# jglaser/metadynamics-plugin

Measured on AMD Instinct MI355X. Metric: particle_cv_evals_per_s, higher is better.
Workload: dtype f32; 1 GPU; 1xMI355X: 10^6 particles, 2 lamellar CVs (8 Fourier modes each), 256^2 bias grid, well-tempered; particles_per_gpu=1000000, particles_global=1000000, n_cv=2, modes_per_cv=8, grid=256x256, stride=1, fast_trig=1, fast_trig_library_default=1, driver=host, mode=single

## Files before the change

metadynamics-plugin_amd/csrc/fused.hip:

```cpp
#include <hip/hip_runtime.h>
#include <hip/hip_ext.h>

#ifdef MTD_STAMPS
__device__ unsigned long long g_stamps[64];
#define MTD_STAMP(slot, cond)                                                   \
    do                                                                          \
        {                                                                       \
        if (cond) g_stamps[slot] = wall_clock64();                              \
        } while (0)
extern "C" int mtd_debug_read_stamps(unsigned long long *host)
    {
    return (int)hipMemcpyFromSymbol(host, HIP_SYMBOL(g_stamps), sizeof(unsigned long long) * 64);
    }
#else
#define MTD_STAMP(slot, cond) do { } while (0)
#endif

#include "lamellar_host.hpp"
#include "metad_host.hpp"
#include "comm_host.hpp"

#include <cstdlib>
#include <cstring>
#include <map>
#include <mutex>
#include <utility>
#include <vector>

namespace
{

using namespace mtd;

constexpr int FCV_THREADS = 512;
constexpr int FCV_UNROLL = 4;
constexpr int FF_THREADS = 256;
constexpr int FF_UNROLL = 2;

template<typename S4, int NCV, bool FAST, bool COMM, bool ORTHO, int U = FCV_UNROLL>
__global__ __launch_bounds__(FCV_THREADS) void k_fused_cv(const LamKArgs a, const S4 *__restrict__ postype, const unsigned int N,
                                                          double *partials, const MetadCfg c,
                                                          const unsigned int n_apply_blocks, const CommK ck)
    {
    __shared__ float s_coeff[MTD_MAX_CV * MTD_MAX_TYPES];
    __shared__ double s_wave[(FCV_THREADS / MTD_WAVE) * NCV];
    __shared__ double s_red[16];
    __shared__ ModeTables s_mt;

    MTD_STAMP(0, blockIdx.x == 0 && threadIdx.x == 0);
    MTD_STAMP(3, blockIdx.x == n_apply_blocks && threadIdx.x == 0);
    if (blockIdx.x < n_apply_blocks)
        {
        const unsigned int b0 = blockIdx.x * FCV_THREADS;
        apply_cells(c, b0, min(c.len, b0 + FCV_THREADS), blockIdx.x == 0, s_red);
        MTD_STAMP(1, blockIdx.x == 0 && threadIdx.x == 0);
        return;
        }
    const unsigned int block_id = blockIdx.x - n_apply_blocks;
    const unsigned int n_blocks = gridDim.x - n_apply_blocks;

    RawGroup<S4, U> first;
    const S4 *src = N ? postype : (const S4 *)partials;
    lam_load_group_nc<S4, U>(src, N ? N : 1u, block_id * FCV_THREADS + threadIdx.x, n_blocks * FCV_THREADS, first);
    const CvTableRegs tab = stage_cv_tables_request(a);
    stage_cv_tables_store(tab, s_coeff, s_mt);
    __syncthreads();
    MTD_STAMP(4, block_id == 0 && threadIdx.x == 0);
    float acc[NCV];
#pragma unroll
    for (int i = 0; i < NCV; ++i) acc[i] = 0.0f;
    lam_cv_accumulate<S4, NCV, FAST, U, ORTHO>(a, postype, N, block_id * FCV_THREADS + threadIdx.x, n_blocks * FCV_THREADS,
                                               s_coeff, s_mt, first, acc);
    MTD_STAMP(5, block_id == 0 && threadIdx.x == 0);
    lam_cv_block_reduce<NCV>(acc, s_wave, partials, block_id);
    MTD_STAMP(6, block_id == 0 && threadIdx.x == 0);
    if (COMM)
        {
        constexpr int NS = NCV < 3 ? NCV : 3;
        if (threadIdx.x < NS)
            ll_store(ck.ll + ((size_t)block_id * NS + threadIdx.x) * 2, ck.seq, partials[block_id * NCV + threadIdx.x]);
        if (block_id != 0 || threadIdx.x >= MTD_WAVE) return;
        double v[3] = { 0.0, 0.0, 0.0 };
        const bool expired = ll_collect_wave<NS>(ck, n_blocks, v);
        MTD_STAMP(7, threadIdx.x == 0);
        double tot[3] = { 0.0, 0.0, 0.0 };
#pragma unroll
        for (int i = 0; i < NS; ++i)
            {
            const double t = wave_sum(v[i]);
            tot[i] = expired ? comm_poison() : t;
            }
        MTD_STAMP(8, threadIdx.x == 0);
        comm_send_wave(ck, tot, NS);
        MTD_STAMP(9, threadIdx.x == 0);
        }
    }

constexpr int FF_STREAM_WAVES = FF_THREADS / MTD_WAVE - 1;
constexpr int FF_STREAM_THREADS = FF_STREAM_WAVES * MTD_WAVE;
constexpr int FF_U = 4;
template<typename S4, int NCV, bool FAST> struct ff_groups { static constexpr int value = 1; };
template<> struct ff_groups<float4, 1, true> { static constexpr int value = 2; };
template<> struct ff_groups<float4, 2, true> { static constexpr int value = 2; };
template<> struct ff_groups<float4, 1, false> { static constexpr int value = 2; };
template<> struct ff_groups<double4, 1, true> { static constexpr int value = 2; };
template<> struct ff_groups<double4, 1, false> { static constexpr int value = 2; };

template<typename S4, int NCV, bool FAST, int GROUPS, bool COMM, bool ORTHO>
__global__ __launch_bounds__(FF_THREADS, 4) void k_fused_force(const LamKArgs a, const S4 *__restrict__ postype, const ForcePtrs out,
                                                            const unsigned int N, const double two_over_n, const MetadCfg c,
                                                            const int deposit, const unsigned int n_grid_blocks, const CommK ck)
    {
    __shared__ ChainResult s_chain;
    __shared__ float s_wcoef[MTD_MAX_CV * MTD_MAX_TYPES];
    __shared__ double s_red[16];
    __shared__ ModeTables s_mt;

    const int wave = threadIdx.x >> 6;
    const int lane = threadIdx.x & 63;
    const bool grid_block = blockIdx.x < n_grid_blocks;
    const unsigned int block_id = blockIdx.x - n_grid_blocks;
    const unsigned int n_blocks = gridDim.x - n_grid_blocks;
    const unsigned int stride = n_blocks * FF_STREAM_THREADS;
    const unsigned int first = block_id * FF_STREAM_THREADS + (wave - 1) * MTD_WAVE + lane;
    const unsigned int first1 = first + FF_U * stride;

    ForceRegs<NCV, FF_U> R, R1;
    MTD_STAMP(16, blockIdx.x == 0 && threadIdx.x == 0);
    MTD_STAMP(24, blockIdx.x == n_grid_blocks && threadIdx.x == 0);
    constexpr int NCH = CHAIN_MAX_CV;
    ChainPre<NCH> pre;
    constexpr bool early = !COMM;
    float4 th = make_float4(0.f, 0.f, 0.f, 0.f), tq = th;
    float tc = 0.0f;
    if (wave == 0)
        {
        if (!grid_block)
            {
            if (lane < (int)a.n_modes)
                {
                th = a.h[lane];
                tq = a.q[lane];
                }
            if (lane < NCV * MTD_MAX_TYPES) tc = a.coeff[lane / MTD_MAX_TYPES][lane % MTD_MAX_TYPES];
            }
        if (early)
            chain_preload<NCH>(c, pre);
        else
            chain_preload<NCH, false>(c, pre);
        }
    RawGroup<S4, FF_U> raw0;
    if (wave != 0 && !grid_block && N) lam_force_request<S4, FF_U>(postype, N, first, stride, raw0);
    if (!grid_block)
        {
        if (wave == 0)
            {
            if (lane < (int)a.n_modes)
                {
                s_mt.h[lane] = th;
                s_mt.q[lane] = tq;
                }
            if (lane < NCV * MTD_MAX_TYPES) s_wcoef[lane] = tc;
            }
        lds_barrier();
        }
    MTD_STAMP(25, blockIdx.x == n_grid_blocks && threadIdx.x == 0);
    if (wave == 0)
        {
        ChainResult r;
        if constexpr (early)
            {
            double vi[3];
#pragma unroll
            for (int i = 0; i < NCH; ++i) vi[i] = (pre.x[i][0] + pre.x[i][1]) + (pre.x[i][2] + pre.x[i][3]);
            r = chain_wave(c, deposit != 0, true, nullptr, nullptr, false, &pre.patch, pre.patch_ok != 0, true, vi[0], vi[1], vi[2]);
            }
        else
            r = chain_wave(c, deposit != 0, true, &ck, nullptr, false, &pre.patch, pre.patch_ok != 0);
        MTD_STAMP(17, blockIdx.x == 0 && threadIdx.x == 0);
        MTD_STAMP(26, blockIdx.x == n_grid_blocks && threadIdx.x == 0);
        if (lane == 0) chain_share(s_chain, r);
        if (!grid_block && lane < NCV * MTD_MAX_TYPES)
            {
            const unsigned int cv = lane / MTD_MAX_TYPES;
            const unsigned int gs = cv < a.n_cv ? a.slot[cv] : 0u;
            const double b = gs == 0 ? r.bias[0] : (gs == 1 ? r.bias[1] : r.bias[2]);
            s_wcoef[lane] = (cv < a.n_cv) ? (float)((double)s_wcoef[lane] * b * two_over_n) : 0.0f;
            }
        }
    else if (!grid_block && N)
        {
        RawGroup<S4, FF_U> raw1;
        if (GROUPS > 1) lam_force_request<S4, FF_U>(postype, N, first1, stride, raw1);
        lam_force_unscaled_from<S4, NCV, FAST, FF_U, ORTHO>(a, N, first, stride, s_mt, raw0, R);
        if (GROUPS > 1) lam_force_unscaled_from<S4, NCV, FAST, FF_U, ORTHO>(a, N, first1, stride, s_mt, raw1, R1);
        MTD_STAMP(27, blockIdx.x == n_grid_blocks && threadIdx.x == 64);
        }
    lds_barrier();
    MTD_STAMP(18, blockIdx.x == 0 && threadIdx.x == 0);
    MTD_STAMP(28, blockIdx.x == n_grid_blocks && threadIdx.x == 64);

    if (grid_block)
        {
        const double2 sums = grid_first_pass_cells_256(c, s_chain, blockIdx.x);
        MTD_STAMP(19, blockIdx.x == 0 && threadIdx.x == 0);
        grid_first_pass_sums_256(c, blockIdx.x, sums, s_red);
        MTD_STAMP(20, blockIdx.x == 0 && threadIdx.x == 0);
        }
    else if (wave != 0 && N)
        {
        lam_force_store<S4, NCV, FF_U>(a, out, first, stride, s_wcoef, R);
        if (GROUPS > 1) lam_force_store<S4, NCV, FF_U>(a, out, first1, stride, s_wcoef, R1);
        MTD_STAMP(29, blockIdx.x == n_grid_blocks && threadIdx.x == 64);
        }

    if (blockIdx.x == 0 && wave == 0) publish_step(c, s_chain, deposit, nullptr, COMM ? &ck : nullptr);
    }

template<typename S4, bool FAST>
__global__ __launch_bounds__(FF_THREADS) void k_fused_force_general(const LamKArgs a, const S4 *__restrict__ postype, const ForcePtrs out,
                                                            const unsigned int N, const double two_over_n, const MetadCfg c,
                                                            const int deposit, const unsigned int n_grid_blocks)
    {
    __shared__ EvalShared sh;
    __shared__ float s_wcoef[MTD_MAX_CV * MTD_MAX_TYPES];
    __shared__ double s_red[16];
    __shared__ ModeTables s_mt;

    load_modes(a, s_mt, true);
    reduce_cv_sources(c, sh.cv, s_red);
    __syncthreads();
    evaluate_bias(c, sh, deposit != 0, true);

    if (blockIdx.x < n_grid_blocks)
        {
        const unsigned int g = blockIdx.x * FF_THREADS + threadIdx.x;
        double s1 = 0.0, s2 = 0.0;
        if (g < c.len)
            {
            const double dV = (c.W * sh.scal) * exp(-gauss_exponent(c, g, sh.cv));
            c.grid_delta[g] = dV;
            unsigned int hd = c.hist_delta[g];
            if (sh.on_grid && g == sh.bin)
                {
                hd += 1;
                c.hist_delta[g] = hd;
                c.sigma_grid_delta[g] += c.det_sigma;
                c.hist_gauss_delta[g] += 1;
                }
            const double R = c.rew[g] + (double)hd;
            c.rew[g] = R;
            s1 = R * dV;
            s2 = R;
            }
        s1 = block_sum(s1, s_red);
        s2 = block_sum(s2, s_red);
        if (threadIdx.x == 0)
            {
            c.gpart[2 * blockIdx.x] = s1;
            c.gpart[2 * blockIdx.x + 1] = s2;
            }
        }

    if (blockIdx.x == 0)
        {
        if (threadIdx.x < c.n_cv)
            {
            c.st->cv[threadIdx.x] = sh.cv[threadIdx.x];
            c.st->bias[threadIdx.x] = sh.bias[threadIdx.x];
            }
        if (threadIdx.x == 0)
            {
            c.st->V = sh.res[0];
            c.st->bin = sh.bin;
            c.st->on_grid = (unsigned int)sh.on_grid;
            if (deposit)
                c.st->scal = sh.scal;
            else
                {
                c.st->w = sh.res[1];
                if (sh.on_grid) c.hist_delta[sh.bin] += 1;
                }
            if (sh.oob[0]) c.st->n_oob += (deposit && c.mode == MTD_MODE_WELL_TEMPERED) ? 2 : 1;
            }
        }
    if (blockIdx.x < n_grid_blocks) return;

    const unsigned int block_id = blockIdx.x - n_grid_blocks;
    const unsigned int n_blocks = gridDim.x - n_grid_blocks;
    for (unsigned int i = threadIdx.x; i < MTD_MAX_CV * MTD_MAX_TYPES; i += blockDim.x)
        {
        const unsigned int cv = i / MTD_MAX_TYPES;
        const double b = cv < a.n_cv ? sh.bias[a.slot[cv]] : 0.0;
        s_wcoef[i] = (float)((double)a.coeff[cv][i % MTD_MAX_TYPES] * b * two_over_n);
        }
    __syncthreads();
    lam_force_pass<S4, FAST, FF_UNROLL>(a, postype, out, N, block_id * FF_THREADS + threadIdx.x, n_blocks * FF_THREADS, s_wcoef, s_mt);
    }

struct ForceProfile
    {
    std::vector<hipEvent_t> ev;
    size_t used = 0;
    };
ForceProfile g_force_profile;
std::mutex g_force_profile_mutex;

bool force_profile_next(hipEvent_t &start, hipEvent_t &stop)
    {
    std::lock_guard<std::mutex> lock(g_force_profile_mutex);
    ForceProfile &p = g_force_profile;
    if (p.used + 2 > p.ev.size()) return false;
    start = p.ev[p.used];
    stop = p.ev[p.used + 1];
    p.used += 2;
    return true;
    }

template<typename F> int with_fused_cv_kernel(int dtype, bool fast, bool ortho, bool comm, unsigned int n_cv, F &&f)
    {
    return dispatch_s4_fast(dtype, fast, [&](auto s4, auto fast_c)
        {
        using S4 = typename decltype(s4)::type;
        constexpr bool FAST = decltype(fast_c)::value;
        return dispatch_bool(ortho, [&](auto ortho_c)
            {
            constexpr bool ORTHO = decltype(ortho_c)::value;
            if (comm)
                return dispatch_count<CHAIN_MAX_CV>(n_cv, [&](auto n) { return f(k_fused_cv<S4, decltype(n)::value, FAST, true, ORTHO>, s4); });
            return dispatch_count<MAXCV>(n_cv, [&](auto n) { return f(k_fused_cv<S4, decltype(n)::value, FAST, false, ORTHO>, s4); });
            });
        });
    }

}

namespace mtd
{
unsigned int resident_capacity(const void *kernel, int threads)
    {
    static std::mutex mu;
    static std::map<std::pair<int, const void *>, unsigned int> cache;
    int per_cu = 0, dev = 0, n_cu = 0;
    if (hipGetDevice(&dev) != hipSuccess)
        {
        (void)hipGetLastError();
        return 0;
        }
    std::lock_guard<std::mutex> lock(mu);
    auto it = cache.find(std::make_pair(dev, kernel));
    if (it != cache.end()) return it->second;
    unsigned int cap = 0;
    if (hipDeviceGetAttribute(&n_cu, hipDeviceAttributeMultiprocessorCount, dev) == hipSuccess &&
        hipOccupancyMaxActiveBlocksPerMultiprocessor(&per_cu, kernel, threads, 0) == hipSuccess)
        cap = (unsigned int)per_cu * (unsigned int)n_cu;
    else
        (void)hipGetLastError();
    cache[std::make_pair(dev, kernel)] = cap;
    return cap;
    }
}

extern "C" {

int mtd_fused_cv_pass(mtd_metad *m, const mtd_lamellar_set *set, unsigned int n_particles, const void *d_postype,
                      int dtype, const mtd_box *global_box, double *d_partials, unsigned int *n_partials,
                      mtd_stream_t stream)
    {
    if (!m) return MTD_ERR_INVALID_ARGUMENT;
    if (m->h_step_err && *m->h_step_err) return MTD_ERR_COMM_TIMEOUT;
    LamKArgs k;
    int rc = fill_kargs(k, set, global_box);
    if (rc) return rc;
    if (!d_partials || !n_partials || (n_particles && !d_postype)) return MTD_ERR_INVALID_ARGUMENT;
    if (dtype != MTD_F32 && dtype != MTD_F64) return MTD_ERR_INVALID_ARGUMENT;
    if (set->n_cv > (unsigned int)MAXCV) return MTD_ERR_UNSUPPORTED;
    hipStream_t s = (hipStream_t)stream;
    const unsigned int blocks = lam_cv_blocks(n_particles);
    *n_partials = blocks;
    const unsigned int n_apply = m->pending_apply ? (m->cfg.len + FCV_THREADS - 1) / FCV_THREADS : 0;
    const bool fast = lam_fast_trig(k) != 0;
    if (m->comm && (set->n_cv > (unsigned int)CHAIN_MAX_CV || set->n_cv != m->cfg.n_cv)) return MTD_ERR_UNSUPPORTED;
    const LamKArgs kd = dense_cv_args(k);
    rc = with_fused_cv_kernel(dtype, fast, k.ortho != 0, m->comm != nullptr, set->n_cv, [&](auto kernel, auto s4) -> int
        {
        using S4 = typename decltype(s4)::type;
        const unsigned int grid = blocks + n_apply;
        CommK ck;
        std::memset(&ck, 0, sizeof(ck));
        if (m->comm)
            {
            if (grid > resident_capacity((const void *)kernel, FCV_THREADS)) return MTD_ERR_UNSUPPORTED;
            const int rcn = comm_next(m->comm, ck);
            if (rcn) return rcn;
            }
        kernel<<<grid, FCV_THREADS, 0, s>>>(kd, (const S4 *)d_postype, n_particles, d_partials, m->cfg, n_apply, ck);
        MTD_LAUNCH_CHECK();
        return MTD_SUCCESS;
        });
    if (rc) return rc;
    m->pending_apply = 0;
    return MTD_SUCCESS;
    }

int mtd_fused_force_pass(mtd_metad *m, const mtd_lamellar_set *set, unsigned int n_particles, const void *d_postype,
                         void *const *d_force, int dtype, unsigned int n_global, const mtd_box *global_box,
                         unsigned int timestep, mtd_stream_t stream)
    {
    if (!m || !set) return MTD_ERR_INVALID_ARGUMENT;
    if (set->n_cv != m->cfg.n_cv) return MTD_ERR_UNSUPPORTED;
    return mtd_fused_force_pass_slots(m, set, nullptr, n_particles, d_postype, d_force, dtype, n_global, global_box, timestep, stream);
    }

int mtd_fused_force_pass_slots(mtd_metad *m, const mtd_lamellar_set *set, const unsigned int *slots, unsigned int n_particles,
                               const void *d_postype, void *const *d_force, int dtype, unsigned int n_global,
                               const mtd_box *global_box, unsigned int timestep, mtd_stream_t stream)
    {
    if (!m) return MTD_ERR_INVALID_ARGUMENT;
    LamKArgs k;
    int rc = fill_kargs(k, set, global_box);
    if (rc) return rc;
    if (!d_force || n_global == 0 || (n_particles && !d_postype)) return MTD_ERR_INVALID_ARGUMENT;
    if (dtype != MTD_F32 && dtype != MTD_F64) return MTD_ERR_INVALID_ARGUMENT;
    if (set->n_cv > m->cfg.n_cv) return MTD_ERR_UNSUPPORTED;
    if (!slots && set->n_cv != m->cfg.n_cv) return MTD_ERR_INVALID_ARGUMENT;
    if (slots)
        {
        if (m->comm) return MTD_ERR_UNSUPPORTED;
        for (unsigned int c = 0; c < set->n_cv; ++c)
            {
            if (slots[c] >= m->cfg.n_cv) return MTD_ERR_INVALID_ARGUMENT;
            k.slot[c] = (unsigned char)slots[c];
            }
        }
    hipStream_t s = (hipStream_t)stream;
    rc = metad_flush(m, s);
    if (rc) return rc;
    ForcePtrs out;
    for (unsigned int c = 0; c < MTD_MAX_CV; ++c) out.f[c] = nullptr;
    for (unsigned int c = 0; c < set->n_cv; ++c)
        {
        if (!d_force[c] && n_particles) return MTD_ERR_INVALID_ARGUMENT;
        out.f[c] = d_force[c];
        }
    const int dep = deposit_due(m, timestep);
    const unsigned int n_grid = dep ? m->cfg.n_gblocks : 0;
    const double two_over_n = 2.0 / (double)n_global;
    const bool fast = lam_fast_trig(k) != 0;
    static const bool force_general = std::getenv("MTD_FUSED_GENERAL") != nullptr;
    CommK ck;
    std::memset(&ck, 0, sizeof(ck));
    if (m->comm)
        {
        if (m->cfg.n_cv > (unsigned int)CHAIN_MAX_CV || force_general) return MTD_ERR_UNSUPPORTED;
        rc = comm_current(m->comm, ck);
        if (rc) return rc;
        }
    if (m->cfg.n_cv <= (unsigned int)CHAIN_MAX_CV && !force_general)
        {
        hipEvent_t ev_start = nullptr, ev_stop = nullptr;
        const bool timed = force_profile_next(ev_start, ev_stop);
        dispatch_s4_fast(dtype, fast, [&](auto s4, auto fast_c)
            {
            using S4 = typename decltype(s4)::type;
            constexpr bool FAST = decltype(fast_c)::value;
            dispatch_count<CHAIN_MAX_CV>(set->n_cv, [&](auto n)
                {
                constexpr int NCV = decltype(n)::value, G = ff_groups<S4, NCV, FAST>::value;
                const unsigned int per_block = FF_STREAM_THREADS * FF_U * G;
                unsigned int fblocks = (n_particles + per_block - 1) / per_block;
                if (fblocks == 0 && n_grid == 0) fblocks = 1;
                const unsigned int grid = n_grid + fblocks;
                dispatch_bool(m->comm != nullptr, [&](auto comm_c)
                    {
                    dispatch_bool(k.ortho != 0, [&](auto ortho_c)
                        {
                        const auto kernel = k_fused_force<S4, NCV, FAST, G, decltype(comm_c)::value, decltype(ortho_c)::value>;
                        if (timed)
                            hipExtLaunchKernelGGL(kernel, dim3(grid), dim3(FF_THREADS), 0, s, ev_start, ev_stop, 0, k, (const S4 *)d_postype, out,
                                                  n_particles, two_over_n, m->cfg, dep, n_grid, ck);
                        else
                            kernel<<<grid, FF_THREADS, 0, s>>>(k, (const S4 *)d_postype, out, n_particles, two_over_n, m->cfg, dep, n_grid, ck);
                        });
                    });
                });
            });
        }
    else
        {
        unsigned int fblocks = lam_force_blocks(n_particles);
        if (n_particles == 0) fblocks = n_grid ? 0 : 1;
        const unsigned int grid = n_grid + fblocks;
        dispatch_s4_fast(dtype, fast, [&](auto s4, auto fast_c)
            {
            using S4 = typename decltype(s4)::type;
            k_fused_force_general<S4, decltype(fast_c)::value><<<grid, FF_THREADS, 0, s>>>(k, (const S4 *)d_postype, out, n_particles, two_over_n,
                                                                                        m->cfg, dep, n_grid);
            });
        }
    MTD_LAUNCH_CHECK();
    m->pending_apply = dep;
    m->w_stale = dep;
    return MTD_SUCCESS;
    }

int mtd_profile_force_begin(unsigned int n_launches)
    {
    std::lock_guard<std::mutex> lock(g_force_profile_mutex);
    ForceProfile &p = g_force_profile;
    for (hipEvent_t e : p.ev) (void)hipEventDestroy(e);
    p.ev.clear();
    p.used = 0;
    for (unsigned int i = 0; i < 2 * n_launches; ++i)
        {
        hipEvent_t e = nullptr;
        MTD_HIP_TRY(hipEventCreate(&e));
        p.ev.push_back(e);
        }
    return MTD_SUCCESS;
    }

int mtd_profile_force_end(double *durations_us, unsigned int capacity, unsigned int *n_out)
    {
    ForceProfile &p = g_force_profile;
    if (!durations_us || !n_out) return MTD_ERR_INVALID_ARGUMENT;
    MTD_HIP_TRY(hipDeviceSynchronize());
    std::lock_guard<std::mutex> lock(g_force_profile_mutex);
    unsigned int n = 0;
    for (size_t i = 0; i + 1 < p.used && n < capacity; i += 2)
        {
        float ms = 0.0f;
        MTD_HIP_TRY(hipEventElapsedTime(&ms, p.ev[i], p.ev[i + 1]));
        durations_us[n++] = 1.0e3 * (double)ms;
        }
    *n_out = n;
    for (hipEvent_t e : p.ev) (void)hipEventDestroy(e);
    p.ev.clear();
    p.used = 0;
    return MTD_SUCCESS;
    }

int mtd_metad_set_comm(mtd_metad *m, mtd_comm *comm)
    {
    if (!m) return MTD_ERR_INVALID_ARGUMENT;
    if (comm && (!comm->connected || m->cfg.n_cv > (unsigned int)CHAIN_MAX_CV || comm->max_doubles < m->cfg.n_cv))
        return comm && !comm->connected ? MTD_ERR_INVALID_ARGUMENT : MTD_ERR_UNSUPPORTED;
    m->comm = comm;
    return MTD_SUCCESS;
    }

}

namespace mtd
{
int fused_grid_step(mtd_metad *m, unsigned int timestep, hipStream_t s)
    {
    if (m->cfg.n_cv > (unsigned int)CHAIN_MAX_CV) return MTD_ERR_UNSUPPORTED;
    int rc = metad_flush(m, s);
    if (rc) return rc;
    LamKArgs k;
    std::memset(&k, 0, sizeof(k));
    k.n_cv = m->cfg.n_cv;
    ForcePtrs out;
    for (unsigned int c = 0; c < MTD_MAX_CV; ++c) out.f[c] = nullptr;
    const int dep = deposit_due(m, timestep);
    const unsigned int n_grid = dep ? m->cfg.n_gblocks : 0;
    const unsigned int grid = n_grid ? n_grid : 1;
    CommK ck;
    std::memset(&ck, 0, sizeof(ck));
    switch (m->cfg.n_cv)
        {
        case 1: k_fused_force<float4, 1, true, 1, false, false><<<grid, FF_THREADS, 0, s>>>(k, nullptr, out, 0, 0.0, m->cfg, dep, n_grid, ck); break;
        case 2: k_fused_force<float4, 2, true, 1, false, false><<<grid, FF_THREADS, 0, s>>>(k, nullptr, out, 0, 0.0, m->cfg, dep, n_grid, ck); break;
        default: k_fused_force<float4, 3, true, 1, false, false><<<grid, FF_THREADS, 0, s>>>(k, nullptr, out, 0, 0.0, m->cfg, dep, n_grid, ck); break;
        }
    MTD_LAUNCH_CHECK();
    m->pending_apply = dep;
    m->w_stale = dep;
    if (dep) announce_pending_apply(m, s);
    return MTD_SUCCESS;
    }
}
```

metadynamics-plugin_amd/csrc/fused_step.hip:

```cpp
#include <hip/hip_runtime.h>

#ifdef MTD_STAMPS
__device__ unsigned long long g_step_stamps[64];
__device__ unsigned long long g_step_block[6][256];
#define MTD_BSTAMP(row) do { g_step_block[row][blockIdx.x] = wall_clock64(); } while (0)
extern "C" int mtd_debug_read_step_blocks(unsigned long long *host)
    {
    return (int)hipMemcpyFromSymbol(host, HIP_SYMBOL(g_step_block), sizeof(unsigned long long) * 6 * 256);
    }
#define MTD_STAMP(slot, cond)                                                   \
    do                                                                          \
        {                                                                       \
        if (cond) g_step_stamps[slot] = wall_clock64();                         \
        } while (0)
extern "C" int mtd_debug_read_step_stamps(unsigned long long *host)
    {
    return (int)hipMemcpyFromSymbol(host, HIP_SYMBOL(g_step_stamps), sizeof(unsigned long long) * 64);
    }
#else
#define MTD_STAMP(slot, cond) do { } while (0)
#define MTD_BSTAMP(row) do { } while (0)
#endif

#include "lamellar_host.hpp"
// ... 55 lines not shown
                    v2f cs;
                    cs.x = cos2pi<FAST>(t.x);
                    cs.y = cos2pi<FAST>(t.y);
                    sum[q] += cs;
                    sum[q] += h.w * ((cs * cs) * 2.0f - (FAST ? 0.99999994f : 1.0f));
                    }
                }
#pragma unroll
            for (int u = 0; u < U; ++u)
                {
                const float w = R.ok[u] ? s_coeff[c * MTD_MAX_TYPES + R.type[u]] : 0.0f;
                acc[c] += w * sum[u / 2][u % 2];
                }
            }
        }
    }

template<int NCV, bool FAST, int U>
__device__ __forceinline__ void step_force_unscaled(const LamKArgs &a, const ModeTables &mt, StepRegs<NCV, U> &R)
    {
#pragma unroll
    for (int c = 0; c < NCV; ++c)
        {
#pragma unroll
        for (int u = 0; u < U; ++u) R.f[u][c][0] = R.f[u][c][1] = R.f[u][c][2] = 0.0f;
        if (c < (int)a.n_cv)
            {
            const unsigned int k1 = a.first[c + 1];
#pragma unroll 4
            for (unsigned int k = a.first[c]; k < k1; ++k)
                {
                const float4 h = mt.h[k];
                const float4 q = mt.q[k];
#pragma unroll
                for (int u = 0; u < U; ++u)
                    {
                    const float s = sin2pi<FAST>(h.x * R.g0[u / 2][u % 2] + h.y * R.g1[u / 2][u % 2] + h.z * R.g2[u / 2][u % 2]);
                    R.f[u][c][0] += q.x * s;
                    R.f[u][c][1] += q.y * s;
                    R.f[u][c][2] += q.z * s;
                    }
                }
            }
        }
    }

template<int NCV> struct ExtraRegs
    {
    float g0, g1, g2;
    int type;
    bool ok;
    float f[NCV][3];
    };

template<int NCV, bool FAST>
__device__ __forceinline__ void step_cv_sums_one(const LamKArgs &a, const float *s_coeff, const ModeTables &mt, const ExtraRegs<NCV> &X,
                                                 float (&acc)[NCV])
    {
#pragma unroll
    for (int c = 0; c < NCV; ++c)
        if (c < (int)a.n_cv)
            {
            float sum = 0.0f;
            const unsigned int k1 = a.first[c] + a.nact[c];
#pragma unroll 4
            for (unsigned int k = a.first[c]; k < k1; ++k)
                {
                const float4 h = mt.h[k];
                const float cs = cos2pi<FAST>(h.x * X.g0 + h.y * X.g1 + h.z * X.g2);
                sum += cs;
                sum += h.w * ((cs * cs) * 2.0f - (FAST ? 0.99999994f : 1.0f));
                }
            acc[c] += (X.ok ? s_coeff[c * MTD_MAX_TYPES + X.type] : 0.0f) * sum;
            }
    }

template<int NCV, bool FAST>
__device__ __forceinline__ void step_force_unscaled_one(const LamKArgs &a, const ModeTables &mt, ExtraRegs<NCV> &X)
    {
#pragma unroll
    for (int c = 0; c < NCV; ++c)
        {
        X.f[c][0] = X.f[c][1] = X.f[c][2] = 0.0f;
        if (c < (int)a.n_cv)
            {
            const unsigned int k1 = a.first[c + 1];
#pragma unroll 4
            for (unsigned int k = a.first[c]; k < k1; ++k)
                {
                const float4 h = mt.h[k];
                const float4 q = mt.q[k];
                const float sn = sin2pi<FAST>(h.x * X.g0 + h.y * X.g1 + h.z * X.g2);
                X.f[c][0] += q.x * sn;
                X.f[c][1] += q.y * sn;
                X.f[c][2] += q.z * sn;
                }
            }
        }
    }

template<typename S4, int NCV, bool FAST, bool COMM>
__global__ __launch_bounds__(FS_THREADS, 1) void k_fused_step(const LamKArgs a, const S4 *__restrict__ postype, const ForcePtrs out,
                                                           const unsigned int N, const unsigned int chunk, const double two_over_n,
                                                           const MetadCfg c, const int deposit, const unsigned int cells_per_block,
                                                           const CommK lk, const CommK ck)
    {
    typedef typename scalar4_traits<S4>::scalar scalar;
    constexpr int NS = NCV;
    __shared__ ChainResult s_chain;
    __shared__ float s_coeff[MTD_MAX_CV * MTD_MAX_TYPES];
    __shared__ float s_wcoef[MTD_MAX_CV * MTD_MAX_TYPES];
    __shared__ double s_wave[FS_WAVES * NCV];
    __shared__ double s_red[2 * FS_WAVES];
    __shared__ double s_avg[2];

    __shared__ ModeTables s_cvt;
    __shared__ ModeTables s_mt;

    const int wave = threadIdx.x >> 6;
    const int lane = threadIdx.x & 63;
    const unsigned int b = blockIdx.x, nb = gridDim.x;
    const unsigned int p0 = b * chunk;
    const unsigned int p1 = min(N, p0 + chunk);
    if (threadIdx.x == 0) MTD_BSTAMP(0);

    MTD_STAMP(0, blockIdx.x == 0 && threadIdx.x == 0); MTD_STAMP(16, blockIdx.x == gridDim.x - 1 && threadIdx.x == 0); MTD_STAMP(32, blockIdx.x == 0 && threadIdx.x == 64);
    StepRegs<NCV, FS_U> R;
    ExtraRegs<NCV> X;
    RawGroup<S4, FS_U> raw;
    S4 raw_x;
    const bool has_extra = wave >= 1 && wave <= (int)FS_EXTRA_WAVES;
    const unsigned int slot0 = (unsigned int)(wave - 1) * MTD_WAVE + lane;
    const unsigned int ix = p0 + FS_U * FS_MAIN + slot0;
    GridPatch patch;
    X.ok = false;
    if (wave == 0)
        {
#pragma unroll
        for (int u = 0; u < FS_U; ++u) R.ok[u] = false;
        patch = chain_prefetch(c);
        }
    else
        {
#pragma unroll
        for (int u = 0; u < FS_U; ++u)
            {
            const unsigned int i = p0 + u * FS_MAIN + slot0;
            R.ok[u] = i < p1;
            if (N) raw.v[u] = postype[R.ok[u] ? i : N - 1];
            }
        X.ok = has_extra && ix < p1;
        if (N && has_extra) raw_x = postype[X.ok ? ix : N - 1];
        }
    load_coeff(a, s_coeff);
    load_modes_cv(a, s_cvt);
    load_modes(a, s_mt, true);
    __syncthreads();

    MTD_STAMP(1, blockIdx.x == 0 && threadIdx.x == 0); MTD_STAMP(17, blockIdx.x == gridDim.x - 1 && threadIdx.x == 0); MTD_STAMP(33, blockIdx.x == 0 && threadIdx.x == 64);
    float acc[NCV];
#pragma unroll
    for (int i = 0; i < NCV; ++i) acc[i] = 0.0f;
    if (wave != 0)
        {
#pragma unroll
        for (int u = 0; u < FS_U; ++u)
            {
            float x0 = 0.0f, x1 = 0.0f, x2 = 0.0f;
            R.type[u] = 0;
            if (N)
                {
                const Particle p = scalar4_traits<S4>::unpack(raw.v[u]);
                project(a, p, x0, x1, x2);
                R.type[u] = p.type;
                }
            R.g0[u / 2][u % 2] = x0;
            R.g1[u / 2][u % 2] = x1;
            R.g2[u / 2][u % 2] = x2;
            }
        step_cv_sums<NCV, FAST, FS_U>(a, s_coeff, s_cvt, R, acc);
        if (has_extra)
            {
            X.g0 = X.g1 = X.g2 = 0.0f;
            X.type = 0;
            if (N)
                {
                const Particle p = scalar4_traits<S4>::unpack(raw_x);
                project(a, p, X.g0, X.g1, X.g2);
                X.type = p.type;
                }
            step_cv_sums_one<NCV, FAST>(a, s_coeff, s_cvt, X, acc);
            }
        }
    MTD_STAMP(2, blockIdx.x == 0 && threadIdx.x == 0); MTD_STAMP(18, blockIdx.x == gridDim.x - 1 && threadIdx.x == 0); MTD_STAMP(34, blockIdx.x == 0 && threadIdx.x == 64);
#pragma unroll
    for (int i = 0; i < NCV; ++i)
        {
        const float v = wave_sum(acc[i]);
        if (lane == 0) s_wave[wave * NCV + i] = (double)v;
        }
    __syncthreads();
    if (threadIdx.x < NS * FS_LL_REPLICAS)
        {
        const int i = threadIdx.x % NS, rep = threadIdx.x / NS;
        double r = 0.0;
        for (int w = 0; w < FS_WAVES; ++w) r += s_wave[w * NCV + i];
        ll_store_column(lk.ll + (size_t)rep * FS_LL_REPLICA_WORDS, FS_LL_PITCH, 2 * i, b, lk.seq, r);
        if (threadIdx.x == 0) MTD_BSTAMP(1);
        }
    __builtin_amdgcn_s_setprio(0);
    MTD_STAMP(3, blockIdx.x == 0 && threadIdx.x == 0); MTD_STAMP(19, blockIdx.x == gridDim.x - 1 && threadIdx.x == 0); MTD_STAMP(35, blockIdx.x == 0 && threadIdx.x == 64);

    double c_wt = 0.0, c_wold = 0.0, c_dV = 0.0;
    const bool closed = deposit != 0 || b != 0;
    if (wave == 0)
        {
        __builtin_amdgcn_s_setprio(3);
        double tot[3] = { 0.0, 0.0, 0.0 };
        bool expired = false;
        if (!COMM || b == 0)
            {
            double v[3] = { 0.0, 0.0, 0.0 };
            CommK rk = lk;
            rk.ll = lk.ll + (size_t)(b % FS_LL_REPLICAS) * FS_LL_REPLICA_WORDS;
            __builtin_amdgcn_s_sleep(FS_FIRST_PROBE_SLEEP);
            expired = ll_collect_columns<NS>(rk, nb, FS_LL_PITCH, 0, v);
#pragma unroll
            for (int i = 0; i < NS; ++i) tot[i] = wave_sum(v[i]);
            if (expired)
#pragma unroll
                for (int i = 0; i < 3; ++i) tot[i] = comm_poison();
            }
        MTD_STAMP(4, blockIdx.x == 0 && threadIdx.x == 0); MTD_STAMP(20, blockIdx.x == gridDim.x - 1 && threadIdx.x == 0);
        if (lane == 0) MTD_BSTAMP(2);
        if (COMM && b == 0) comm_send_wave(ck, tot, NS);
        const ChainResult r = chain_wave(c, deposit != 0, closed, COMM ? &ck : nullptr, COMM ? nullptr : tot, b == 0 && deposit != 0, &patch);
        c_wt = r.c_wt; c_wold = r.c_wold; c_dV = r.c_dV;
        MTD_STAMP(5, blockIdx.x == 0 && threadIdx.x == 0); MTD_STAMP(21, blockIdx.x == gridDim.x - 1 && threadIdx.x == 0);
        if (lane == 0) MTD_BSTAMP(3);
        if (lane == 0) chain_share(s_chain, r);
        for (unsigned int i = lane; i < NCV * MTD_MAX_TYPES; i += MTD_WAVE)
            {
            const unsigned int cv = i / MTD_MAX_TYPES;
            const double bf = cv == 0 ? r.bias[0] : (cv == 1 ? r.bias[1] : r.bias[2]);
            s_wcoef[i] = (cv < a.n_cv) ? (float)((double)a.coeff[cv][i % MTD_MAX_TYPES] * bf * two_over_n) : 0.0f;
            }
        __builtin_amdgcn_s_setprio(0);
        }
    else
        {
        step_force_unscaled<NCV, FAST, FS_U>(a, s_mt, R);
        if (has_extra) step_force_unscaled_one<NCV, FAST>(a, s_mt, X);
        }
    MTD_STAMP(6, blockIdx.x == 0 && threadIdx.x == 0); MTD_STAMP(22, blockIdx.x == gridDim.x - 1 && threadIdx.x == 0); MTD_STAMP(38, blockIdx.x == 0 && threadIdx.x == 64);
    lds_barrier();
    MTD_STAMP(7, blockIdx.x == 0 && threadIdx.x == 0); MTD_STAMP(23, blockIdx.x == gridDim.x - 1 && threadIdx.x == 0); MTD_STAMP(39, blockIdx.x == 0 && threadIdx.x == 64);

    auto store_forces = [&]()
        {
#pragma unroll
        for (int cvi = 0; cvi < NCV; ++cvi)
            {
            if (cvi < (int)a.n_cv)
                {
                S4 *f = (S4 *)out.f[cvi];
#pragma unroll
                for (int u = 0; u < FS_U; ++u)
                    if (R.ok[u])
                        {
                        const float w = s_wcoef[cvi * MTD_MAX_TYPES + R.type[u]];
                        nt_store(scalar4_traits<S4>::make((scalar)(R.f[u][cvi][0] * w), (scalar)(R.f[u][cvi][1] * w), (scalar)(R.f[u][cvi][2] * w), (scalar)0),
                                 &f[p0 + u * FS_MAIN + slot0]);
                        }
                if (X.ok)
                    {
                    const float w = s_wcoef[cvi * MTD_MAX_TYPES + X.type];
                    nt_store(scalar4_traits<S4>::make((scalar)(X.f[cvi][0] * w), (scalar)(X.f[cvi][1] * w), (scalar)(X.f[cvi][2] * w), (scalar)0), &f[ix]);
                    }
                }
            }
        };

    const bool failed = s_chain.failed != 0;
    MTD_STAMP(8, blockIdx.x == 0 && threadIdx.x == 0); MTD_STAMP(24, blockIdx.x == gridDim.x - 1 && threadIdx.x == 0); MTD_STAMP(40, blockIdx.x == 0 && threadIdx.x == 64);
    const bool dep = deposit != 0 && !failed;
    const unsigned int cell0 = min(c.len, b * cells_per_block), cell1 = min(c.len, cell0 + cells_per_block);
    const bool grid_wave = dep && cell0 + (unsigned int)wave * MTD_WAVE < cell1;
    if (!grid_wave) store_forces();
    double avg_dV = 0.0;
    bool grid_expired = false;
    if (dep)
        {
        double s1 = 0.0, s2 = 0.0;
        for (unsigned int g = cell0 + threadIdx.x; g < cell1; g += FS_THREADS)
            {
            const double2 t = grid_first_pass_cell(c, s_chain, g);
            s1 += t.x;
            s2 += t.y;
            }
        s1 = wave_sum(s1);
        s2 = wave_sum(s2);
        if (lane == 0)
            {
            s_red[2 * wave] = s1;
            s_red[2 * wave + 1] = s2;
            }
        lds_barrier();
        if (threadIdx.x < 2 * FS_LL_REPLICAS)
            {
            const unsigned int i = threadIdx.x & 1, rep = threadIdx.x >> 1;
            double t = 0.0;
            for (int w = 0; w < FS_WAVES; ++w) t += s_red[2 * w + i];
            ll_store_column(lk.ll + (size_t)rep * FS_LL_REPLICA_WORDS, FS_LL_PITCH, 2 * (CHAIN_MAX_CV + i), b, lk.seq, t);
            if (threadIdx.x == 0) MTD_BSTAMP(4);
            }
        if (grid_wave) store_forces();
    MTD_STAMP(9, blockIdx.x == 0 && threadIdx.x == 0); MTD_STAMP(25, blockIdx.x == gridDim.x - 1 && threadIdx.x == 0); MTD_STAMP(41, blockIdx.x == 0 && threadIdx.x == 64);
        if (wave == 0)
            {
            double v[3] = { 0.0, 0.0, 0.0 };
            CommK rk = lk;
            rk.ll = lk.ll + (size_t)(b % FS_LL_REPLICAS) * FS_LL_REPLICA_WORDS;
            const bool ex = ll_collect_columns<2>(rk, nb, FS_LL_PITCH, 2 * CHAIN_MAX_CV, v);
            const double t1 = wave_sum(v[0]), t2 = wave_sum(v[1]);
            if (lane == 0)
                {
                s_avg[0] = t1 / t2;
                s_avg[1] = ex ? 1.0 : 0.0;
                }
            }
        lds_barrier();
        avg_dV = s_avg[0];
    MTD_STAMP(10, blockIdx.x == 0 && threadIdx.x == 0); MTD_STAMP(26, blockIdx.x == gridDim.x - 1 && threadIdx.x == 0); MTD_STAMP(42, blockIdx.x == 0 && threadIdx.x == 64);
        grid_expired = s_avg[1] != 0.0;
        if (!grid_expired)
            for (unsigned int g = cell0 + threadIdx.x; g < cell1; g += FS_THREADS)
                {
                const double dV = c.grid_delta[g];
                const double fac = exp(-(dV - avg_dV) / c.temp);
                c.rew[g] *= fac;
                c.weight[g] /= fac;
                c.grid[g] += dV;
                c.sigma_grid[g] += c.sigma_grid_delta[g];
                c.hist[g] += c.hist_delta[g];
                c.hist_gauss[g] += c.hist_gauss_delta[g];
                c.grid_delta[g] = 0.0;
                c.sigma_grid_delta[g] = 0.0;
                c.hist_delta[g] = 0;
                c.hist_gauss_delta[g] = 0;
                }
        if (blockIdx.x == 0 && threadIdx.x == 0) c.st->patch_valid = 0;
        }

    if (threadIdx.x == 0) MTD_BSTAMP(5);
    MTD_STAMP(11, blockIdx.x == 0 && threadIdx.x == 0); MTD_STAMP(27, blockIdx.x == gridDim.x - 1 && threadIdx.x == 0); MTD_STAMP(43, blockIdx.x == 0 && threadIdx.x == 64);
    if (b == 0 && wave == 0)
        {
        double w_now = s_chain.w;
        if (dep && !grid_expired)
            {
            const int n_term = 1 << c.n_cv;
            double term = 0.0;
            if (lane < n_term && c_wt != 0.0) term = c_wt * (c_wold / exp(-(c_dV - avg_dV) / c.temp));
            w_now = 0.0;
            for (int q = 0; q < n_term; ++q) w_now += __shfl(term, q, MTD_WAVE);
            }
        if (lane < (int)c.n_cv)
            {
            c.st->cv[lane] = lane == 0 ? s_chain.cv[0] : (lane == 1 ? s_chain.cv[1] : s_chain.cv[2]);
            c.st->bias[lane] = lane == 0 ? s_chain.bias[0] : (lane == 1 ? s_chain.bias[1] : s_chain.bias[2]);
            }
        if (lane == 0)
            {
            c.st->V = s_chain.V;
            c.st->failed = (failed || grid_expired) ? 1u : 0u;
            c.st->bin = s_chain.bin;
            c.st->on_grid = (unsigned int)s_chain.on_grid;
            if (failed)
                c.st->w = s_chain.V;
            else if (deposit)
                {
                c.st->scal = s_chain.scal;
                if (!grid_expired)
                    {
                    c.st->w = w_now;
                    c.st->avg_dV = avg_dV;
                    c.st->num_gaussians += 1;
                    }
                }
// ... 181 lines not shown
```

metadynamics-plugin_amd/csrc/mesh.hip:

```cpp
#include "mtd_device.hpp"
#include "comm_host.hpp"
#include "exact_div.hpp"
#include "lamellar_host.hpp"
#include "metad_host.hpp"

#include <algorithm>
#include <cmath>
#include <type_traits>
#include <cstdio>
#include <cstdlib>
#include <cstring>
#include <map>
#include <mutex>
#include <new>
#include <utility>
#include <vector>

namespace
{

using namespace mtd;


struct MeshGeom
// ... 1235 lines not shown
    {
    static constexpr int E = (TP_HMAX + NT - 1) / NT;
    double v[E];
    unsigned int dst[E];
    };

template<int NT>
__device__ __forceinline__ void tile_stage_load(TileStage<NT> &st, const unsigned int tid, const unsigned int n_rows, const unsigned int wxn,
                                                const unsigned int *s_grow, const unsigned short *s_lrow, const unsigned short *s_gx,
                                                const double *__restrict__ inv)
    {
    const unsigned int n_img = n_rows * wxn;
    static_assert(TP_HMAX < 12288 && TP_HMAX * (TP_X + 2) <= (1 << 20), "multiply-shift division of the flat image index");
    const unsigned int inv_w = ((1u << 20) + wxn - 1) / wxn;
#pragma unroll
    for (int e = 0; e < TileStage<NT>::E; ++e)
        {
        const unsigned int idx = tid + e * NT;
        st.v[e] = 0.0;
        st.dst[e] = ~0u;
        if (idx < n_img)
            {
            const unsigned int row = (idx * inv_w) >> 20, lx = idx - row * wxn;
            st.v[e] = inv[s_grow[row] + s_gx[lx]];
            st.dst[e] = s_lrow[row] + lx;
            }
        }
    }

template<int NT>
__device__ __forceinline__ void tile_stage_store(const TileStage<NT> &st, double *s_inv)
    {
#pragma unroll
    for (int e = 0; e < TileStage<NT>::E; ++e)
        if (st.dst[e] != ~0u) s_inv[st.dst[e]] = st.v[e];
    }

template<typename S4>
__device__ __forceinline__ void tile_force_of(const MeshGeom &g, const TileGeom &tg, const double *s_inv, const double *s_mode,
                                              const double *__restrict__ mode, const double4 &cur, const double s, S4 *__restrict__ force)
    {
    typedef typename scalar4_traits<S4>::scalar scalar;
    const unsigned int bt = (unsigned int)__double2hiint(cur.w);
    const uint2 cib = make_uint2((unsigned int)__double2loint(cur.w), bt & 0xffffu);
    const double a = mode_of(s_mode, mode, bt >> 16), sx = cur.x, sy = cur.y, sz = cur.z;
    double wxv[3], wyv[3], wzv[3], dxv[3], dyv[3], dzv[3];
    tsc3_deriv(sx, wxv, dxv);
    tsc3_deriv(sy, wyv, dyv);
    tsc3_deriv(sz, wzv, dzv);
    double g1 = 0.0, g2 = 0.0, g3 = 0.0;
#pragma unroll
    for (int k = 0; k < 3; ++k)
        {
        double pd = 0.0, pdy = 0.0, pw = 0.0;
#pragma unroll
        for (int j = 0; j < 3; ++j)
            {
#ifdef MTD_EXP_LDS_NOCONFLICT
            const unsigned int row = (threadIdx.x + 3 * TF_THREADS * (k * 3 + j)) % 6000u + 0u * cib.y;
            const double r0 = s_inv[row], r1 = s_inv[row + TF_THREADS], r2 = s_inv[(row + 2 * TF_THREADS) % 6144u];
#else
            const unsigned int row = cib.y + tg.hx * (j + tg.hy * k);
            const double r0 = s_inv[row], r1 = s_inv[row + 1], r2 = s_inv[row + 2];
#endif
            const double aw = wxv[0] * r0 + wxv[1] * r1 + wxv[2] * r2;
            const double ad = dxv[0] * r0 + dxv[1] * r1 + dxv[2] * r2;
            pd += wyv[j] * ad;
            pdy += dyv[j] * aw;
            pw += wyv[j] * aw;
            }
        g1 += wzv[k] * pd;
        g2 += wzv[k] * pdy;
        g3 += dzv[k] * pw;
        }
    const double c1 = -(double)g.nx * a * g1, c2 = -(double)g.ny * a * g2, c3 = -(double)g.nz * a * g3;
    const double fx = (c1 * g.binv[0][0] + c2 * g.binv[1][0] + c3 * g.binv[2][0]) * s;
    const double fy = (c1 * g.binv[0][1] + c2 * g.binv[1][1] + c3 * g.binv[2][1]) * s;
    const double fz = (c1 * g.binv[0][2] + c2 * g.binv[1][2] + c3 * g.binv[2][2]) * s;
    force[cib.x] = scalar4_traits<S4>::make((scalar)fx, (scalar)fy, (scalar)fz, (scalar)0);
    }

template<typename S4>
__global__ __launch_bounds__(TF_THREADS) void k_tile_forces(const MeshGeom g, const TileGeom tg, const TileLists L,
                                                            const double *__restrict__ mode, const double4 *__restrict__ packed,
                                                            const double *__restrict__ inv, S4 *__restrict__ force,
                                                            const double *__restrict__ d_bias, const double bias_host,
                                                            const double two_over_n, const unsigned int n_types)
    {
    __shared__ double s_inv[TP_HMAX];
    __shared__ double s_mode[TP_MODE_LDS];
    stage_modes(s_mode, mode, n_types);
    const unsigned int per_xcd = (tg.n_tiles + 7) / 8;
    const unsigned int t = (blockIdx.x & 7u) * per_xcd + (blockIdx.x >> 3);
    if ((blockIdx.x >> 3) >= per_xcd || t >= tg.n_tiles) return;
    const unsigned int tix = t % tg.ntx, tiy = (t / tg.ntx) % tg.nty, tiz = t / (tg.ntx * tg.nty);
    const int x0 = tix * tg.tx, y0 = tiy * tg.ty, z0 = tiz * tg.tz;
    TILE_STAMP(1, 0);
    const unsigned int n_all = L.count[(size_t)t * L.cstride];
    const unsigned int q0 = L.first[t], q1 = q0 + (L.cap ? min(n_all, L.cap[t]) : n_all);
    const unsigned int n_ovf = L.ovf_count ? *L.ovf_count : 0u;
    if (n_all == 0) return;
    unsigned int q = q0 + threadIdx.x;
    const unsigned int q_last = q1 > q0 ? q1 - 1 : q0;
    double4 pk = packed[min(q, q_last)];
    const unsigned int wxn = min(tg.tx, g.nx - x0) + 2, wyn = min(tg.ty, g.ny - y0) + 2, wzn = min(tg.tz, g.nz - z0) + 2;
    constexpr int TF_MAXROWS = (TP_Y + 2) * (TP_Z + 2);
    __shared__ unsigned int s_grow[TF_MAXROWS];
    __shared__ unsigned short s_lrow[TF_MAXROWS];
    __shared__ unsigned short s_gx[TP_X + 2];
    const unsigned int n_rows = wyn * wzn;
    for (unsigned int r = threadIdx.x; r < n_rows; r += TF_THREADS)
        {
        const unsigned int lz = r / wyn, ly = r - lz * wyn;
        int gy = y0 + (int)ly - 1, gz = z0 + (int)lz - 1;
        gy = gy < 0 ? gy + (int)g.ny : (gy >= (int)g.ny ? gy - (int)g.ny : gy);
        gz = gz < 0 ? gz + (int)g.nz : (gz >= (int)g.nz ? gz - (int)g.nz : gz);
        s_grow[r] = g.nx * ((unsigned int)gy + g.ny * (unsigned int)gz);
        s_lrow[r] = (unsigned short)(tg.hx * (ly + tg.hy * lz));
        }
    if (threadIdx.x < wxn)
        {
        int gx = x0 + (int)threadIdx.x - 1;
        gx = gx < 0 ? gx + (int)g.nx : (gx >= (int)g.nx ? gx - (int)g.nx : gx);
        s_gx[threadIdx.x] = (unsigned short)gx;
        }
    __syncthreads();
    {
    TileStage<TF_THREADS> st;
    tile_stage_load<TF_THREADS>(st, threadIdx.x, n_rows, wxn, s_grow, s_lrow, s_gx, inv);
    tile_stage_store<TF_THREADS>(st, s_inv);
    }
    __syncthreads();
    TILE_STAMP(1, 1);
    const double bias = d_bias ? *d_bias : bias_host;
    const double s = two_over_n * bias;
    auto force_of = [&](const double4 &cur) { tile_force_of<S4>(g, tg, s_inv, s_mode, mode, cur, s, force); };
    while (q < q1)
        {
        const double4 cur = pk;
        const unsigned int qn = q + TF_THREADS;
        pk = packed[min(qn, q_last)];
        force_of(cur);
        if (q == q0 + threadIdx.x) TILE_STAMP(1, 2);
        q = qn;
        }
    for (unsigned int k = threadIdx.x; k < n_ovf; k += TF_THREADS)
        if (L.ovf_tile[k] == t) force_of(packed[L.ovf_base + k]);
    TILE_STAMP(1, 3);
    }

constexpr int TFC_STREAM_THREADS = TF_THREADS - MTD_WAVE;
constexpr int TFC_U = 4;

template<typename S4, int NCV, bool FAST>
__global__ __launch_bounds__(TF_THREADS, 4) void k_tile_forces_chain(const MeshGeom g, const TileGeom tg, const TileLists L,
                                                                  const double *__restrict__ mode, const double4 *__restrict__ packed,
                                                                  const double *__restrict__ inv, S4 *__restrict__ force,
                                                                  const double two_over_n, const unsigned int n_types, const unsigned int mesh_slot,
                                                                  const mtd::LamKArgs a, const S4 *__restrict__ postype, const mtd::ForcePtrs out,
                                                                  const unsigned int N, const mtd::MetadCfg c, const int deposit,
                                                                  const unsigned int n_grid_blocks)
    {
    using namespace mtd;
    static_assert(TF_THREADS >= 320, "threads 0 .. 255 of a block take a grid block's cells, wave 0 runs the chain");
    __shared__ double s_inv[TP_HMAX];
    __shared__ double s_mode[TP_MODE_LDS];
    __shared__ ChainResult s_chain;
    __shared__ float s_wcoef[MTD_MAX_CV * MTD_MAX_TYPES];
    __shared__ double s_red[8];
    __shared__ ModeTables s_mt;
    constexpr int TF_MAXROWS = (TP_Y + 2) * (TP_Z + 2);
    __shared__ unsigned int s_grow[TF_MAXROWS];
    __shared__ unsigned short s_lrow[TF_MAXROWS];
    __shared__ unsigned short s_gx[TP_X + 2];
    const int wave = threadIdx.x >> 6, lane = threadIdx.x & 63;

    constexpr int NCH = CHAIN_MAX_CV;
    ChainPre<NCH> pre;
    float4 th = make_float4(0.f, 0.f, 0.f, 0.f), tq = th;
    float tc = 0.0f;
    if (wave == 0)
        {
        if (lane < (int)a.n_modes)
            {
            th = a.h[lane];
            tq = a.q[lane];
            }
        if (lane < NCV * MTD_MAX_TYPES) tc = a.coeff[lane / MTD_MAX_TYPES][lane % MTD_MAX_TYPES];
        chain_preload<NCH>(c, pre);
        }
    const unsigned int sid = threadIdx.x - MTD_WAVE;
    const unsigned int stride = gridDim.x * TFC_STREAM_THREADS;
    const unsigned int first = blockIdx.x * TFC_STREAM_THREADS + sid;
    RawGroup<S4, TFC_U> raw0;
    if (wave != 0 && N) lam_force_request<S4, TFC_U>(postype, N, first, stride, raw0);
    const unsigned int per_xcd = (tg.n_tiles + 7) / 8;
    const unsigned int t = (blockIdx.x & 7u) * per_xcd + (blockIdx.x >> 3);
    const bool has_tile = (blockIdx.x >> 3) < per_xcd && t < tg.n_tiles;
    const unsigned int tt = has_tile ? t : 0u;
    const unsigned int tix = tt % tg.ntx, tiy = (tt / tg.ntx) % tg.nty, tiz = tt / (tg.ntx * tg.nty);
    const int x0 = tix * tg.tx, y0 = tiy * tg.ty, z0 = tiz * tg.tz;
    const unsigned int n_all = has_tile ? L.count[(size_t)tt * L.cstride] : 0u;
    const unsigned int q0 = L.first[tt], q1 = q0 + (L.cap ? min(n_all, L.cap[tt]) : n_all);
    const unsigned int n_ovf = L.ovf_count ? *L.ovf_count : 0u;
    const bool work = n_all != 0;
    unsigned int q = q0 + threadIdx.x;
    const unsigned int q_last = q1 > q0 ? q1 - 1 : q0;
    double4 pk = make_double4(0.0, 0.0, 0.0, 0.0);
    if (work) pk = packed[min(q, q_last)];
    stage_modes(s_mode, mode, n_types);
    const unsigned int wxn = min(tg.tx, g.nx - x0) + 2, wyn = min(tg.ty, g.ny - y0) + 2, wzn = min(tg.tz, g.nz - z0) + 2;
    const unsigned int n_rows = wyn * wzn;
    if (work)
        {
        for (unsigned int r = threadIdx.x; r < n_rows; r += TF_THREADS)
            {
            const unsigned int lz = r / wyn, ly = r - lz * wyn;
            int gy = y0 + (int)ly - 1, gz = z0 + (int)lz - 1;
            gy = gy < 0 ? gy + (int)g.ny : (gy >= (int)g.ny ? gy - (int)g.ny : gy);
            gz = gz < 0 ? gz + (int)g.nz : (gz >= (int)g.nz ? gz - (int)g.nz : gz);
            s_grow[r] = g.nx * ((unsigned int)gy + g.ny * (unsigned int)gz);
            s_lrow[r] = (unsigned short)(tg.hx * (ly + tg.hy * lz));
            }
        if (threadIdx.x < wxn)
            {
            int gx = x0 + (int)threadIdx.x - 1;
            gx = gx < 0 ? gx + (int)g.nx : (gx >= (int)g.nx ? gx - (int)g.nx : gx);
            s_gx[threadIdx.x] = (unsigned short)gx;
            }
        }
    if (wave == 0)
        {
        if (lane < (int)a.n_modes)
            {
            s_mt.h[lane] = th;
            s_mt.q[lane] = tq;
            }
        if (lane < NCV * MTD_MAX_TYPES) s_wcoef[lane] = tc;
        }
    lds_barrier();

    ForceRegs<NCV, TFC_U> R;
    if (wave == 0)
        {
        double vi[3];
#pragma unroll
        for (int i = 0; i < NCH; ++i) vi[i] = (pre.x[i][0] + pre.x[i][1]) + (pre.x[i][2] + pre.x[i][3]);
        const ChainResult r = chain_wave(c, deposit != 0, true, nullptr, nullptr, false, &pre.patch, pre.patch_ok != 0, true, vi[0], vi[1], vi[2]);
        if (lane == 0) chain_share(s_chain, r);
        if (lane < NCV * MTD_MAX_TYPES)
            {
            const unsigned int cv = lane / MTD_MAX_TYPES;
            const unsigned int gs = cv < a.n_cv ? a.slot[cv] : 0u;
            const double b = gs == 0 ? r.bias[0] : (gs == 1 ? r.bias[1] : r.bias[2]);
            s_wcoef[lane] = (cv < a.n_cv) ? (float)((double)s_wcoef[lane] * b * two_over_n) : 0.0f;
            }
        }
    else
        {
        TileStage<TFC_STREAM_THREADS> st;
        if (work) tile_stage_load<TFC_STREAM_THREADS>(st, sid, n_rows, wxn, s_grow, s_lrow, s_gx, inv);
        if (N) lam_force_unscaled_from<S4, NCV, FAST, TFC_U>(a, N, first, stride, s_mt, raw0, R);
        if (work) tile_stage_store<TFC_STREAM_THREADS>(st, s_inv);
        }
    __syncthreads();

    if (wave != 0 && N)
        {
        lam_force_store<S4, NCV, TFC_U>(a, out, first, stride, s_wcoef, R);
        for (unsigned int f = first + TFC_U * stride; f < N; f += TFC_U * stride)
            {
            lam_force_unscaled<S4, NCV, FAST, TFC_U>(a, postype, N, f, stride, s_mt, R);
            lam_force_store<S4, NCV, TFC_U>(a, out, f, stride, s_wcoef, R);
            }
        }
    if (blockIdx.x < n_grid_blocks) grid_first_pass_256(c, s_chain, blockIdx.x, s_red);
    if (blockIdx.x == 0 && wave == 0) publish_step(c, s_chain, deposit);
    if (!work) return;
    const double bias = mesh_slot == 0 ? s_chain.bias[0] : (mesh_slot == 1 ? s_chain.bias[1] : s_chain.bias[2]);
    const double s = two_over_n * bias;
    while (q < q1)
        {
        const double4 cur = pk;
        const unsigned int qn = q + TF_THREADS;
        pk = packed[min(qn, q_last)];
        tile_force_of<S4>(g, tg, s_inv, s_mode, mode, cur, s, force);
        q = qn;
        }
    for (unsigned int k = threadIdx.x; k < n_ovf; k += TF_THREADS)
        if (L.ovf_tile[k] == tt) tile_force_of<S4>(g, tg, s_inv, s_mode, mode, packed[L.ovf_base + k], s, force);
    }

constexpr int FFT_THREADS = 256;

__device__ __forceinline__ void dft_direct(const double2 *in, double2 *out, const double2 *__restrict__ twiddle, const unsigned int n,
                                           const unsigned int tile, const int inverse)
    {
    for (unsigned int idx = threadIdx.x; idx < n * tile; idx += FFT_THREADS)
        {
        const unsigned int k = idx / tile, t = idx % tile;
        double re = 0.0, im = 0.0;
        unsigned int r = 0;
        for (unsigned int p = 0; p < n; ++p)
            {
            double2 w = twiddle[r];
            if (inverse) w.y = -w.y;
            const double2 v = in[p * tile + t];
            re += v.x * w.x - v.y * w.y;
            im += v.x * w.y + v.y * w.x;
            r += k;
            if (r >= n) r -= n;
            }
        out[k * tile + t] = make_double2(re, im);
        }
    __syncthreads();
    }

__device__ __forceinline__ unsigned int lds_slot(const unsigned int p, const unsigned int log2n)
    {
    return log2n ? (__brev(p) >> (32 - log2n)) : p;
    }

__device__ __forceinline__ double2 cmul(const double2 a, const double2 w) { return make_double2(a.x * w.x - a.y * w.y, a.x * w.y + a.y * w.x); }
__device__ __forceinline__ double2 cadd(const double2 a, const double2 b) { return make_double2(a.x + b.x, a.y + b.y); }
__device__ __forceinline__ double2 csub(const double2 a, const double2 b) { return make_double2(a.x - b.x, a.y - b.y); }

__device__ __forceinline__ void fft_dit_pow2(double2 *s, const double2 *__restrict__ twiddle, const unsigned int log2n,
                                             const unsigned int log2tile, const int inverse, const unsigned int stride)
    {
    const unsigned int n = 1u << log2n, tile = 1u << log2tile, tmask = tile - 1;
    unsigned int log2len = 1;
    if (log2n & 1)
        {
        for (unsigned int idx = threadIdx.x; idx < (n >> 1) << log2tile; idx += FFT_THREADS)
            {
            const unsigned int t = idx & tmask, bf = idx >> log2tile;
            const unsigned int i0 = bf << 1;
            const double2 u = s[i0 * stride + t], v = s[(i0 + 1) * stride + t];
            s[i0 * stride + t] = cadd(u, v);
            s[(i0 + 1) * stride + t] = csub(u, v);
            }
        __syncthreads();
        log2len = 2;
        }
    for (; log2len < log2n + 1; log2len += 2)
        {
        const unsigned int log2half = log2len - 1, half = 1u << log2half;
        for (unsigned int idx = threadIdx.x; idx < (n >> 2) << log2tile; idx += FFT_THREADS)
            {
            const unsigned int t = idx & tmask, bf = idx >> log2tile;
            const unsigned int grp = bf >> log2half, j = bf & (half - 1);
            const unsigned int ia = (grp << (log2len + 1)) + j;
            double2 w1 = twiddle[j << (log2n - log2len)];
            double2 w2 = twiddle[j << (log2n - log2len - 1)];
            if (inverse)
                {
                w1.y = -w1.y;
                w2.y = -w2.y;
                }
            double2 *pa = s + ia * stride + t;
            const unsigned int sh = half * stride;
            const double2 a = pa[0], b = cmul(pa[sh], w1), c = pa[2 * sh], d = cmul(pa[3 * sh], w1);
            const double2 a1 = cadd(a, b), b1 = csub(a, b), c1 = cmul(cadd(c, d), w2), d1 = cmul(csub(c, d), w2);
            const double2 d1r = inverse ? make_double2(-d1.y, d1.x) : make_double2(d1.y, -d1.x);
            pa[0] = cadd(a1, c1);
            pa[2 * sh] = csub(a1, c1);
            pa[sh] = cadd(b1, d1r);
            pa[3 * sh] = csub(b1, d1r);
            }
        __syncthreads();
        }
    }

__device__ __forceinline__ void fft_dif_pow2_inverse(double2 *s, const double2 *__restrict__ twiddle, const unsigned int log2n,
                                                     const unsigned int log2tile)
    {
    const unsigned int n = 1u << log2n, tile = 1u << log2tile, tmask = tile - 1;
    int log2len = (int)log2n;
    for (; log2len >= 2; log2len -= 2)
        {
        const unsigned int log2q = log2len - 2, q = 1u << log2q;
        for (unsigned int idx = threadIdx.x; idx < (n >> 2) << log2tile; idx += FFT_THREADS)
            {
            const unsigned int t = idx & tmask, bf = idx >> log2tile;
            const unsigned int grp = bf >> log2q, j = bf & (q - 1);
            const unsigned int ia = (grp << log2len) + j;
            double2 wa = twiddle[j << (log2n - log2len)];
            double2 w2 = twiddle[j << (log2n - log2len + 1)];
            wa.y = -wa.y;
            w2.y = -w2.y;
            double2 *pa = s + (ia << log2tile) + t;
            const unsigned int sh = q << log2tile;
            const double2 a = pa[0], b = pa[sh], c = pa[2 * sh], d = pa[3 * sh];
            const double2 a1 = cadd(a, c), c1 = cmul(csub(a, c), wa);
            const double2 bd = csub(b, d);
            const double2 b1 = cadd(b, d), d1 = cmul(make_double2(-bd.y, bd.x), wa);
            pa[0] = cadd(a1, b1);
            pa[sh] = cmul(csub(a1, b1), w2);
            pa[2 * sh] = cadd(c1, d1);
            pa[3 * sh] = cmul(csub(c1, d1), w2);
            }
        __syncthreads();
        }
    if (log2len == 1)
        {
        for (unsigned int idx = threadIdx.x; idx < (n >> 1) << log2tile; idx += FFT_THREADS)
            {
            const unsigned int t = idx & tmask, bf = idx >> log2tile;
            const unsigned int i0 = bf << 1;
            const double2 u = s[(i0 << log2tile) + t], v = s[((i0 + 1) << log2tile) + t];
            s[(i0 << log2tile) + t] = cadd(u, v);
            s[((i0 + 1) << log2tile) + t] = csub(u, v);
            }
        __syncthreads();
        }
    }

__device__ __forceinline__ unsigned int ilog2_dev(const unsigned int v) { return 31u - (unsigned int)__clz((int)v); }

template<bool REAL_INPUT, bool REAL_OUTPUT>
__global__ __launch_bounds__(FFT_THREADS) void k_fft_lines(const double *__restrict__ real_in, double2 *__restrict__ data,
                                                           double *__restrict__ real_out,
                                                           const double2 *__restrict__ twiddle, const unsigned int n,
                                                           const unsigned int log2n, const unsigned int tile,
                                                           const unsigned int elem_stride, const unsigned int line_stride,
                                                           const unsigned int tiles_per_row, const unsigned int row_stride,
                                                           const int inverse, const int p_fastest)
    {
    extern __shared__ __attribute__((aligned(16))) char smem[];
    double2 *s = (double2 *)smem;
// ... 2141 lines not shown
        MTD_LAUNCH_CHECK();
        rc = launch_fft_y(m, m->d_f, 0, s);
        if (rc) return rc;
        m->last_forward = 0;
        }
    const FftPass pz = fft_z_pass(m);
    SlabArgs none;
    std::memset(&none, 0, sizeof(none));
    const unsigned int tpb = fft_z_tpb(pz);
    unsigned int z_blocks_whole = pz.n_blocks / tpb;
    static const bool edge_off = [] { const char *e = std::getenv("MTD_FFT_Z_EDGE"); return !(e && e[0] == '1'); }();
    const unsigned int hx_cols = m->nx / 2 + 1;
    const bool z_edge = !edge_off && tpb == 1 && pz.tile > 1 && hx_cols % pz.tile == 1 && (hx_cols / pz.tile + 1) == pz.tiles_per_row && m->ny >= pz.tile;
    if (z_edge)
        {
        const unsigned int full = hx_cols / pz.tile, n_regular = full * m->ny, n_edge = (m->ny + pz.tile - 1) / pz.tile;
        z_blocks_whole = n_regular + n_edge;
        k_fft_z_spectral<false, 1><<<z_blocks_whole, FFT_THREADS, fft_lds_bytes(pz.n, pz.tile), s>>>(
            g, m->d_f, m->d_g, pz.tw, ilog2(pz.n), pz.tile, full, m->d_mode_sq, (double)n_global, m->d_itab, m->d_cv_partials, none, m->keep_fourier,
            n_regular, full * pz.tile);
        }
    else if (tpb == 3)
        k_fft_z_spectral<false, 3><<<z_blocks_whole, FFT_THREADS, fft_lds_bytes(pz.n, pz.tile), s>>>(
            g, m->d_f, m->d_g, pz.tw, ilog2(pz.n), pz.tile, pz.tiles_per_row, m->d_mode_sq, (double)n_global, m->d_itab, m->d_cv_partials, none, m->keep_fourier, 0xffffffffu, 0u);
    else if (tpb == 2)
        k_fft_z_spectral<false, 2><<<z_blocks_whole, FFT_THREADS, fft_lds_bytes(pz.n, pz.tile), s>>>(
            g, m->d_f, m->d_g, pz.tw, ilog2(pz.n), pz.tile, pz.tiles_per_row, m->d_mode_sq, (double)n_global, m->d_itab, m->d_cv_partials, none, m->keep_fourier, 0xffffffffu, 0u);
    else
        k_fft_z_spectral<false, 1><<<z_blocks_whole, FFT_THREADS, fft_lds_bytes(pz.n, pz.tile), s>>>(
            g, m->d_f, m->d_g, pz.tw, ilog2(pz.n), pz.tile, pz.tiles_per_row, m->d_mode_sq, (double)n_global, m->d_itab, m->d_cv_partials, none, m->keep_fourier, 0xffffffffu, 0u);
    m->fourier_valid = m->keep_fourier;
    bool fold_cv = false;
    unsigned int n_folded = 0;
    if (m->cv_event) MTD_HIP_TRY(hipEventRecord(m->cv_event, s));
    MTD_LAUNCH_CHECK();
    if (xy)
        {
        const unsigned int xy_blocks = m->nz * XY_PARTS;
        fold_cv = !m->cv_event && z_blocks_whole > xy_blocks && z_blocks_whole <= 64 * xy_blocks;
        XYSplit xs_i;
        size_t xs_lds = 0;
        const char *split_env = std::getenv("MTD_FFT_SPLIT");
        const bool split = !(split_env && split_env[0] == '0') && xy_split_plan(m, xs_i, xs_lds);
        if (split)
            k_fft_xy_inverse_split<<<xy_blocks, XY_THREADS, xs_lds, s>>>(m->d_g, m->d_inv, m->d_tw[0], m->d_tw[1], xs_i, m->d_cv_partials,
                                                                         fold_cv ? z_blocks_whole : 0u, m->d_cv_folded);
        else
            k_fft_xy_inverse<<<xy_blocks, XY_THREADS, xy_lds_i, s>>>(m->d_g, m->d_inv, m->d_tw[0], m->d_tw[1], xy_i, m->d_cv_partials,
                                                                     fold_cv ? z_blocks_whole : 0u, m->d_cv_folded);
        MTD_LAUNCH_CHECK();
        if (fold_cv) n_folded = xy_blocks;
        }
    else
        {
        rc = launch_fft_y(m, m->d_g, 1, s);
        if (rc) return rc;
        k_fft_x_c2r<<<x_blocks, FFT_THREADS, x_lds, s>>>(m->d_g, m->d_inv, m->d_tw[0], m->nx, ilog2(m->nx), x_tile, m->hxp, n_lines);
        MTD_LAUNCH_CHECK();
        }
    *d_partials = fold_cv ? m->d_cv_folded : m->d_cv_partials;
    *n_partials = fold_cv ? n_folded : z_blocks_whole;
    return MTD_SUCCESS;
    }

int mtd_mesh_compute_cv(mtd_mesh *m, unsigned int n_particles, const void *d_postype, int dtype, const mtd_box *box,
                        unsigned int n_global, const double **d_partials, unsigned int *n_partials, mtd_stream_t stream)
    {
    if (!m || !d_partials || !n_partials || n_global == 0) return MTD_ERR_INVALID_ARGUMENT;
    XYPlan xy_probe;
    XYTiles tl_probe;
    size_t lds_probe = 0;
    static const bool xy_off = [] { const char *e = std::getenv("MTD_FFT_XY"); return e && e[0] == '0'; }();
    const bool from_tiles = m->tile_path && !xy_off && xy_plan(m, 0, xy_probe, lds_probe) && xy_tiles_ok(m, tl_probe) && m->tg.ty &&
                            m->nx == 128 && XY_THREADS == 512 && xy_probe.pb == 32 && 16 % m->tg.ty == 0 && (2 * xy_probe.pb) % m->tg.ty == 0;
    int rc = mesh_assign_local(m, n_particles, d_postype, dtype, box, stream, !from_tiles);
    if (rc) return rc;
    return mtd_mesh_spectral(m, box, n_global, d_partials, n_partials, stream);
    }

int mtd_mesh_forces(mtd_mesh *m, unsigned int n_particles, const void *d_postype, void *d_force, int dtype, const mtd_box *box,
                    unsigned int n_global, const double *d_bias, double bias_host, mtd_stream_t stream)
    {
    if (!m || n_global == 0 || (n_particles && (!d_postype || !d_force))) return MTD_ERR_INVALID_ARGUMENT;
    if (dtype != MTD_F32 && dtype != MTD_F64) return MTD_ERR_INVALID_ARGUMENT;
    if (n_particles == 0) return MTD_SUCCESS;
    MeshGeom g;
    int rc = fill_geom(g, m, box);
    if (rc) return rc;
    hipStream_t s = (hipStream_t)stream;
    unsigned int blocks = (n_particles + 255) / 256;
    if (blocks > 4096) blocks = 4096;
    const double two_over_n = 2.0 / (double)n_global;
    if (n_particles != m->n_last) return MTD_ERR_INVALID_ARGUMENT;
    if (m->tile_path)
        {
        if (dtype == MTD_F32)
            k_tile_forces<float4><<<8 * ((m->tg.n_tiles + 7) / 8), TF_THREADS, 0, s>>>(g, m->tg, m->lists, m->d_mode, m->d_packed, m->d_inv, (float4 *)d_force, d_bias, bias_host, two_over_n, m->n_types);
        else
            k_tile_forces<double4><<<8 * ((m->tg.n_tiles + 7) / 8), TF_THREADS, 0, s>>>(g, m->tg, m->lists, m->d_mode, m->d_packed, m->d_inv, (double4 *)d_force, d_bias, bias_host, two_over_n, m->n_types);
        MTD_LAUNCH_CHECK();
        return MTD_SUCCESS;
        }
    if (dtype == MTD_F32)
        k_mesh_forces<float4><<<blocks, 256, 0, s>>>(g, n_particles, m->d_idcell, m->d_packed, m->d_inv, (float4 *)d_force, d_bias, bias_host, two_over_n);
    else
        k_mesh_forces<double4><<<blocks, 256, 0, s>>>(g, n_particles, m->d_idcell, m->d_packed, m->d_inv, (double4 *)d_force, d_bias, bias_host, two_over_n);
    MTD_LAUNCH_CHECK();
    return MTD_SUCCESS;
    }

int mtd_mesh_forces_update_bias(mtd_mesh *mesh, mtd_metad *m, unsigned int mesh_slot, const mtd_lamellar_set *set, const unsigned int *slots,
                                unsigned int n_particles, const void *d_postype, void *d_force_mesh, void *const *d_force_lamellar,
                                int dtype, unsigned int n_global, const mtd_box *box, unsigned int timestep, mtd_stream_t stream)
    {
    const unsigned int n_lam = set ? set->n_cv : 0u;
    if (!mesh || !m || n_global == 0 || !box || (n_lam && (!slots || !d_force_lamellar))) return MTD_ERR_INVALID_ARGUMENT;
    if (dtype != MTD_F32 && dtype != MTD_F64) return MTD_ERR_INVALID_ARGUMENT;
    if (n_particles == 0 || !d_postype || !d_force_mesh) return MTD_ERR_UNSUPPORTED;
    static const bool off = [] { const char *e = std::getenv("MTD_MESH_FORCE_MERGED"); return e && e[0] == '0'; }();
    if (off || !mesh->tile_path || m->comm) return MTD_ERR_UNSUPPORTED;
    if (m->cfg.n_cv > (unsigned int)mtd::CHAIN_MAX_CV || mesh_slot >= m->cfg.n_cv) return MTD_ERR_UNSUPPORTED;
    if (n_lam > 3 || n_lam >= m->cfg.n_cv) return MTD_ERR_UNSUPPORTED;
    if (n_particles != mesh->n_last) return MTD_ERR_INVALID_ARGUMENT;
    if (m->h_step_err && *m->h_step_err) return MTD_ERR_COMM_TIMEOUT;
    mtd::LamKArgs k;
    int rc = MTD_SUCCESS;
    if (n_lam)
        rc = mtd::fill_kargs(k, set, box);
    else
        std::memset(&k, 0, sizeof(k));
    if (rc) return rc;
    for (unsigned int cv = 0; cv < n_lam; ++cv)
        {
        if (slots[cv] >= m->cfg.n_cv || slots[cv] == mesh_slot) return MTD_ERR_INVALID_ARGUMENT;
        if (!d_force_lamellar[cv]) return MTD_ERR_INVALID_ARGUMENT;
        k.slot[cv] = (unsigned char)slots[cv];
        }
    const int dep = deposit_due(m, timestep);
    const unsigned int n_grid = dep ? m->cfg.n_gblocks : 0;
    const unsigned int blocks = 8 * ((mesh->tg.n_tiles + 7) / 8);
    if (n_grid > blocks) return MTD_ERR_UNSUPPORTED;
    if ((unsigned long long)blocks * TFC_STREAM_THREADS * TFC_U >= (1ull << 31)) return MTD_ERR_UNSUPPORTED;
    MeshGeom g;
    rc = fill_geom(g, mesh, box);
    if (rc) return rc;
    hipStream_t s = (hipStream_t)stream;
    rc = mtd::metad_flush(m, s);
    if (rc) return rc;
    mtd::ForcePtrs out;
    for (unsigned int cv = 0; cv < MTD_MAX_CV; ++cv) out.f[cv] = cv < n_lam ? d_force_lamellar[cv] : nullptr;
    const double two_over_n = 2.0 / (double)n_global;
    const bool fast = n_lam ? mtd::lam_fast_trig(k) != 0 : true;
    const unsigned int n_stream = n_lam ? n_particles : 0u;
#define MTD_LAUNCH_TFC(S4, NCV, FASTV) \
    k_tile_forces_chain<S4, NCV, FASTV><<<blocks, TF_THREADS, 0, s>>>(g, mesh->tg, mesh->lists, mesh->d_mode, mesh->d_packed, mesh->d_inv, (S4 *)d_force_mesh, \
        two_over_n, mesh->n_types, mesh_slot, k, (const S4 *)d_postype, out, n_stream, m->cfg, dep, n_grid)
#define MTD_LAUNCH_TFC_NCV(S4, FASTV) \
    switch (n_lam) { case 0: case 1: MTD_LAUNCH_TFC(S4, 1, FASTV); break; case 2: MTD_LAUNCH_TFC(S4, 2, FASTV); break; default: MTD_LAUNCH_TFC(S4, 3, FASTV); break; }
    if (dtype == MTD_F32)
        {
        if (fast) { MTD_LAUNCH_TFC_NCV(float4, true) } else { MTD_LAUNCH_TFC_NCV(float4, false) }
        }
    else
        {
        if (fast) { MTD_LAUNCH_TFC_NCV(double4, true) } else { MTD_LAUNCH_TFC_NCV(double4, false) }
        }
#undef MTD_LAUNCH_TFC_NCV
#undef MTD_LAUNCH_TFC
    MTD_LAUNCH_CHECK();
    m->pending_apply = dep;
    m->w_stale = dep;
    if (dep) mtd::announce_pending_apply(m, s);
    return MTD_SUCCESS;
    }

int mtd_mesh_slab_bytes(const mtd_mesh *m, unsigned int world, size_t *bytes)
    {
    if (!m || !bytes || world == 0 || world > MTD_COMM_MAX_RANKS) return MTD_ERR_INVALID_ARGUMENT;
    if (m->nz % world || m->ny % world) return MTD_ERR_UNSUPPORTED;
    bytes[0] = sizeof(double) * (size_t)m->M;
    bytes[1] = sizeof(double2) * (size_t)(m->nz / world) * m->ny * m->hxp;
    bytes[2] = sizeof(double2) * (size_t)m->nz * (m->ny / world) * m->hxp;
    bytes[3] = sizeof(double) * (size_t)(m->nz / world) * m->ny * m->nx;
    return MTD_SUCCESS;
    }

int mtd_mesh_slab_attach(mtd_mesh *m, mtd_comm *comm, void *const *rho_peers, void *const *f_peers, void *const *g_peers,
                         void *const *inv_peers)
    {
    if (!m || !comm || !rho_peers || !f_peers || !g_peers || !inv_peers) return MTD_ERR_INVALID_ARGUMENT;
    const unsigned int world = mtd_comm_world(comm);
    if (m->nz % world || m->ny % world || !m->tile_path) return MTD_ERR_UNSUPPORTED;
    m->slab_comm = comm;
    m->slab_world = world;
    m->slab_rank = mtd_comm_rank(comm);
    for (unsigned int r = 0; r < world; ++r)
        {
        if (!rho_peers[r] || !f_peers[r] || !g_peers[r] || !inv_peers[r]) return MTD_ERR_INVALID_ARGUMENT;
        m->slab_rho[r] = rho_peers[r]; m->slab_f[r] = f_peers[r]; m->slab_g[r] = g_peers[r]; m->slab_inv[r] = inv_peers[r];
        }
    if (!m->d_slab_rho) MTD_HIP_TRY(hipMalloc((void **)&m->d_slab_rho, sizeof(double) * (size_t)(m->nz / world) * m->ny * m->nx));
    if (!m->d_slab_sum)
        {
        MTD_HIP_TRY(hipMalloc((void **)&m->d_slab_sum, sizeof(double) * 2));
        MTD_HIP_TRY(hipMemset(m->d_slab_sum, 0, sizeof(double) * 2));
        }
    return MTD_SUCCESS;
    }

int mtd_mesh_slab_compute_cv(mtd_mesh *m, unsigned int n_particles, const void *d_postype, int dtype, const mtd_box *box,
                             unsigned int n_global, const double **d_cv_sum, mtd_stream_t stream)
    {
    if (!m || !m->slab_comm || !d_cv_sum || n_global == 0) return MTD_ERR_INVALID_ARGUMENT;
    MeshGeom g;
    int rc = fill_geom(g, m, box);
    if (rc) return rc;
    hipStream_t s = (hipStream_t)stream;
    const unsigned int W = m->slab_world, r = m->slab_rank, nzl = m->nz / W, nyl = m->ny / W;
    const size_t slab_cells = (size_t)nzl * m->ny * m->nx;
    double *rho_x = (double *)m->slab_rho[r];
    double2 *f_x = (double2 *)m->slab_f[r], *g_x = (double2 *)m->slab_g[r];
    double *inv_x = (double *)m->slab_inv[r];
    PeerPtrs pp;
    auto peers_of = [&](const void *const *src) { std::memset(&pp, 0, sizeof(pp)); for (unsigned int q = 0; q < W; ++q) pp.p[q] = src[q]; };

    rc = mesh_assign_local(m, n_particles, d_postype, dtype, box, stream);
    if (rc) return rc;
    k_copy_doubles<<<1024, 256, 0, s>>>(m->d_rho, rho_x, (size_t)m->M);
    MTD_LAUNCH_CHECK();
    rc = mtd_comm_allreduce_small(m->slab_comm, m->d_slab_sum + 1, 1, stream);
    if (rc) return rc;
    peers_of(m->slab_rho);
    k_slab_pull_rho<<<1024, 256, 0, s>>>(pp, W, (size_t)r * slab_cells, slab_cells, m->d_slab_rho);
    MTD_LAUNCH_CHECK();
    const unsigned int n_lines = m->ny * nzl;
    unsigned int x_pairs = 8;
    while (x_pairs > 1 && fft_x_lds_bytes(m->nx, x_pairs) > 64 * 1024) x_pairs >>= 1;
    const unsigned int x_tile = 2 * x_pairs, x_blocks = (n_lines + x_tile - 1) / x_tile;
    const size_t x_lds = fft_x_lds_bytes(m->nx, x_pairs);
    k_fft_x_r2c<<<x_blocks, FFT_THREADS, x_lds, s>>>(m->d_slab_rho, m->d_f, m->d_tw[0], m->nx, ilog2(m->nx), x_tile, m->hxp, n_lines);
    MTD_LAUNCH_CHECK();
    FftPass py = fft_y_pass(m);
    py.n_blocks = py.tiles_per_row * nzl;
    k_fft_lines<false, false><<<py.n_blocks, FFT_THREADS, fft_lds_bytes(py.n, py.tile), s>>>(
        nullptr, m->d_f, nullptr, py.tw, py.n, ilog2(py.n), py.tile, py.elem_stride, py.line_stride, py.tiles_per_row, py.row_stride, 0, py.p_fastest);
    MTD_LAUNCH_CHECK();
    k_copy_doubles<<<1024, 256, 0, s>>>((const double *)m->d_f, (double *)f_x, 2 * (size_t)nzl * m->ny * m->hxp);
    MTD_LAUNCH_CHECK();
    rc = mtd_comm_allreduce_small(m->slab_comm, m->d_mode_sq, 1, stream);
    if (rc) return rc;
    const FftPass pz = fft_z_pass(m);
    SlabArgs sl;
    std::memset(&sl, 0, sizeof(sl));
    for (unsigned int q = 0; q < W; ++q) sl.f[q] = (const double2 *)m->slab_f[q];
    sl.world = W; sl.nz_loc = nzl; sl.ny_loc = nyl; sl.y0 = r * nyl;
    const unsigned int z_blocks = pz.tiles_per_row * nyl;
    k_fft_z_spectral<true, 1><<<z_blocks, FFT_THREADS, fft_lds_bytes(pz.n, pz.tile), s>>>(
        g, nullptr, g_x, pz.tw, ilog2(pz.n), pz.tile, pz.tiles_per_row, m->d_mode_sq, (double)n_global, m->d_itab, m->d_cv_partials, sl, 0, 0xffffffffu, 0u);
    m->fourier_valid = 0;
    MTD_LAUNCH_CHECK();
    rc = mtd_reduce_partials(m->d_cv_partials, z_blocks, 1, 1, 1.0, 0.0, m->d_slab_sum, stream);
    if (rc) return rc;
    rc = mtd_comm_allreduce_small(m->slab_comm, m->d_slab_sum, 1, stream);
    if (rc) return rc;
    peers_of(m->slab_g);
    k_slab_pull_g<<<1024, 256, 0, s>>>(pp, r * nzl, nzl, m->ny, nyl, m->hxp, m->d_g);
    MTD_LAUNCH_CHECK();
    k_fft_lines<false, false><<<py.n_blocks, FFT_THREADS, fft_lds_bytes(py.n, py.tile), s>>>(
        nullptr, m->d_g, nullptr, py.tw, py.n, ilog2(py.n), py.tile, py.elem_stride, py.line_stride, py.tiles_per_row, py.row_stride, 1, py.p_fastest);
    MTD_LAUNCH_CHECK();
    k_fft_x_c2r<<<x_blocks, FFT_THREADS, x_lds, s>>>(m->d_g, inv_x, m->d_tw[0], m->nx, ilog2(m->nx), x_tile, m->hxp, n_lines);
    MTD_LAUNCH_CHECK();
    rc = mtd_comm_allreduce_small(m->slab_comm, m->d_slab_sum + 1, 1, stream);
    if (rc) return rc;
    peers_of(m->slab_inv);
    k_slab_pull_inv<<<1024, 256, 0, s>>>(pp, W, slab_cells, m->d_inv);
    MTD_LAUNCH_CHECK();
    *d_cv_sum = m->d_slab_sum;
    return MTD_SUCCESS;
    }

int mtd_mesh_set_table(mtd_mesh *m, const double *K, const double *d_K, unsigned int n, double k_min, double k_max)
    {
    if (!m || !K || !d_K || n < 2) return MTD_ERR_INVALID_ARGUMENT;
    if (k_min < 0 || k_max < 0 || k_max <= k_min) return MTD_ERR_INVALID_ARGUMENT;
    if (m->d_table) MTD_HIP_TRY(hipFree(m->d_table));
    m->d_table = nullptr;
    MTD_HIP_TRY(hipMalloc((void **)&m->d_table, sizeof(double) * 2 * n));
    m->d_table_d = m->d_table + n;
    MTD_HIP_TRY(hipMemcpy(m->d_table, K, sizeof(double) * n, hipMemcpyHostToDevice));
    MTD_HIP_TRY(hipMemcpy(m->d_table_d, d_K, sizeof(double) * n, hipMemcpyHostToDevice));
    m->n_table = n;
    m->k_min = k_min;
    m->k_max = k_max;
    m->delta_k = (k_max - k_min) / (double)(n - 1);
    return MTD_SUCCESS;
    }

int mtd_mesh_set_use_table(mtd_mesh *m, int use_table)
    {
    if (!m) return MTD_ERR_INVALID_ARGUMENT;
    if (use_table && !m->d_table) return MTD_ERR_INVALID_ARGUMENT;
    m->use_table = use_table ? 1 : 0;
    return MTD_SUCCESS;
    }

static int log_scratch(mtd_mesh *m)
    {
    if (!m->d_log_scratch) MTD_HIP_TRY(hipMalloc((void **)&m->d_log_scratch, sizeof(double) * 8 * 256));
    return MTD_SUCCESS;
    }
// ... 121 lines not shown
```

metadynamics-plugin_amd/csrc/metad_device.hpp:

```cpp
#pragma once

#include "mtd_device.hpp"
#include "comm_device.hpp"
#include "exact_div.hpp"

#ifndef MTD_STAMP
#define MTD_STAMP(slot, cond) do { } while (0)
#endif

namespace mtd
{

constexpr int MAXCV = MTD_METAD_MAX_CV;
constexpr int GRID_THREADS = 256;
constexpr int MAX_POINTS = 2 * MAXCV + 2;
constexpr int MAX_TERMS = 1 << MAXCV;

struct CvSource
    {
    const double *partials;
    unsigned int n_partials, stride, offset, _pad;
    double scale, shift;
    };

struct MetadState
    {
    double cv[MAXCV];
    double bias[MAXCV];
    double V;
    double w;
    double scal;
    double avg_dV;
    unsigned int num_gaussians;
    unsigned int n_oob;
    unsigned int bin;
    unsigned int on_grid;
    unsigned int failed;
    unsigned int _pad;
    int patch_valid;
    int patch_org[3];
    int guess_org[3];
    int _pad2;
    double zero;
    double patch_v[216];
    };

struct MetadCfg
    {
    unsigned int n_cv, len;
    unsigned int lengths[MAXCV];
    unsigned int factors[MAXCV];
    double cv_min[MAXCV], cv_max[MAXCV], delta[MAXCV];
    double sigma_inv[MAXCV * MAXCV];
    double W, T_shift, temp, det_sigma;
    int mode, _pad;
    double *grid, *grid_delta, *rew, *weight, *sigma_grid, *sigma_grid_delta;
    unsigned int *hist, *hist_delta, *hist_gauss, *hist_gauss_delta;
    MetadState *st;
    double *gpart;
    unsigned int n_gblocks;
    int fastdiv;
    double rdelta[3], rdelta2[3], rT_shift;
    CvSource src[MAXCV];
    };

__device__ __forceinline__ void decode(const MetadCfg &c, unsigned int idx, unsigned int *coords)
    {
    unsigned int rest = idx;
    for (int i = (int)c.n_cv - 1; i >= 0; --i)
        {
        coords[i] = rest / c.factors[i];
        rest -= coords[i] * c.factors[i];
        }
    }

__device__ __forceinline__ double gauss_exponent(const MetadCfg &c, unsigned int idx, const double *s)
    {
    unsigned int coords[MAXCV];
    decode(c, idx, coords);
    double d[MAXCV];
    for (unsigned int i = 0; i < c.n_cv; ++i)
        {
        const double val_i = c.cv_min[i] + coords[i] * c.delta[i];
        d[i] = val_i - s[i];
        }
    double gauss_exp = 0.0;
    for (unsigned int i = 0; i < c.n_cv; ++i)
        for (unsigned int j = 0; j < c.n_cv; ++j)
            {
            const double sij = c.sigma_inv[i * c.n_cv + j];
            gauss_exp += d[i] * d[j] * (1.0 / 2.0) * (sij * sij);
            }
    return gauss_exp;
    }

__device__ __forceinline__ bool bin_of(const MetadCfg &c, const double *val, unsigned int &idx)
    {
    bool on_grid = true;
    unsigned int r = 0;
    for (unsigned int i = 0; i < c.n_cv; ++i)
        {
        const double q = (val[i] - c.cv_min[i]) / c.delta[i];
        if (!(q > -1.0) || !(q < 4294967296.0))
            {
            on_grid = false;
            continue;
            }
        const unsigned int coord = (unsigned int)q;
        if (coord >= c.lengths[i]) on_grid = false;
        r += coord * c.factors[i];
        }
    idx = r;
    return on_grid;
    }

__device__ __forceinline__ bool interp_corner(const MetadCfg &c, const double *val, unsigned int bits, unsigned int &cell,
                                              double &weight)
    {
    double t = 1.0;
    unsigned int idx = 0;
    for (unsigned int i = 0; i < c.n_cv; ++i)
        {
        const double v = val[i];
        if (v < c.cv_min[i] || v >= c.cv_max[i]) return false;
        int lower = (int)((v - c.cv_min[i]) / c.delta[i]);
        int upper = lower + 1;
        if (upper >= (int)c.lengths[i])
            {
            lower--;
            upper--;
            }
        const double lower_bound = c.cv_min[i] + c.delta[i] * lower;
        const double upper_bound = c.cv_min[i] + c.delta[i] * upper;
        const double rel = (v - lower_bound) / (upper_bound - lower_bound);
        if (bits & (1u << i))
            {
            idx += (unsigned int)lower * c.factors[i];
            t *= (1.0 - rel);
            }
        else
            {
            idx += (unsigned int)upper * c.factors[i];
            t *= rel;
            }
        }
    cell = idx;
    weight = t;
    return true;
    }

__device__ __forceinline__ void reduce_cv_sources(const MetadCfg &c, double *s_cv, double *s_tmp)
    {
    const int lane = threadIdx.x & 63;
    const int wave = threadIdx.x >> 6;
    const int n_waves = blockDim.x >> 6;
    for (unsigned int i = 0; i < c.n_cv; ++i)
        {
// ... 106 lines not shown
        for (int b = 0; b < n_term; ++b) res += sh.wt[p][b] * sh.val[p][b];
        sh.res[p] = res;
        }
    __syncthreads();
    if (threadIdx.x < n)
        {
        const unsigned int i = threadIdx.x;
        const double s = sh.cv[i];
        const double delta = c.delta[i];
        double b;
        if (s - delta < c.cv_min[i])
            b = (sh.res[3 + 2 * i] - sh.res[0]) / delta;
        else if (s + delta > c.cv_max[i])
            b = (sh.res[0] - sh.res[2 + 2 * i]) / delta;
        else
            b = (sh.res[3 + 2 * i] - sh.res[2 + 2 * i]) / (2.0 * delta);
        sh.bias[i] = b;
        }
    __syncthreads();
    }

__device__ __forceinline__ void apply_cells(const MetadCfg &c, const unsigned int cell_begin, const unsigned int cell_end,
                                            const bool first, double *s_red)
    {
    if (c.st->failed) return;
    double s1 = 0.0, s2 = 0.0;
    for (unsigned int b = threadIdx.x; b < c.n_gblocks; b += blockDim.x)
        {
        s1 += c.gpart[2 * b];
        s2 += c.gpart[2 * b + 1];
        }
    s1 = block_sum(s1, s_red);
    s2 = block_sum(s2, s_red);
    const double avg_dV = s1 / s2;

    const unsigned int g = cell_begin + threadIdx.x;
    if (g < cell_end)
        {
        const double dV = c.grid_delta[g];
        const double fac = exp(-(dV - avg_dV) / c.temp);
        c.rew[g] *= fac;
        c.weight[g] /= fac;
        const double g_new = c.grid[g] + dV;
        c.grid[g] = g_new;
        if (c.n_cv <= 3)
            {
            unsigned int rest = g;
            int slot = 0;
            bool in = true;
            for (int i = (int)c.n_cv - 1; i >= 0; --i)
                {
                const unsigned int co = rest / c.factors[i];
                rest -= co * c.factors[i];
                const int o = (int)co - c.st->guess_org[i];
                in = in && o >= 0 && o < 6;
                slot += o * (i == 0 ? 1 : (i == 1 ? 6 : 36));
                }
            if (in) c.st->patch_v[slot] = g_new;
            }
        const double sgd = c.sigma_grid_delta[g];
        if (sgd != 0.0)
            {
            c.sigma_grid[g] += sgd;
            c.sigma_grid_delta[g] = 0.0;
            }
        const unsigned int hd = c.hist_delta[g], hgd = c.hist_gauss_delta[g];
        if (hd)
            {
            c.hist[g] += hd;
            c.hist_delta[g] = 0;
            }
        if (hgd)
            {
            c.hist_gauss[g] += hgd;
            c.hist_gauss_delta[g] = 0;
            }
        c.grid_delta[g] = 0.0;
        }
    if (first && threadIdx.x == 0)
        {
        c.st->patch_org[0] = c.st->guess_org[0];
        c.st->patch_org[1] = c.st->guess_org[1];
        c.st->patch_org[2] = c.st->guess_org[2];
        c.st->patch_valid = c.n_cv <= 3 ? 1 : 0;
        c.st->avg_dV = avg_dV;
        c.st->num_gaussians += 1;
        }
    }

struct ChainResult
    {
    double cv[3];
    double bias[3];
    double scal, V, w;
    unsigned int bin;
    int on_grid, oob;
    int failed;
    double c_wt, c_wold, c_dV;
    };

constexpr int CHAIN_MAX_CV = 3;

struct GridPatch
    {
    double v[4];
    int org[CHAIN_MAX_CV];
    };

__device__ __forceinline__ GridPatch chain_prefetch(const MetadCfg &c)
    {
    const int lane = threadIdx.x & 63;
    const int n = (int)c.n_cv;
    GridPatch gp;
    int total = 1;
#pragma unroll
    for (int i = 0; i < CHAIN_MAX_CV; ++i)
        {
        gp.org[i] = 0;
        if (i < n)
            {
            const double s = c.st->cv[i];
            double q = (s - c.cv_min[i]) / c.delta[i];
            if (!(q > 0.0)) q = 0.0;
            if (q > (double)c.lengths[i]) q = (double)c.lengths[i];
            gp.org[i] = (int)q - 2;
            total *= 6;
            }
        }
#pragma unroll
    for (int r = 0; r < 4; ++r)
        {
        gp.v[r] = 0.0;
        const int slot = lane + 64 * r;
        if (slot < total)
            {
            int rest = slot;
            bool in = true;
            unsigned int cell = 0;
#pragma unroll
            for (int i = 0; i < CHAIN_MAX_CV; ++i)
                if (i < n)
                    {
                    const int coord = gp.org[i] + rest % 6;
                    rest /= 6;
                    in = in && coord >= 0 && coord < (int)c.lengths[i];
                    cell += (unsigned int)coord * c.factors[i];
                    }
            if (in) gp.v[r] = c.grid[cell];
            }
        }
    return gp;
    }

template<int NCH> struct ChainPre
    {
    double x[NCH][4];
    GridPatch patch;
    int patch_ok;
    };

template<int NCH, bool SUMS = true>
__device__ __forceinline__ void chain_preload(const MetadCfg &c, ChainPre<NCH> &p)
    {
    const unsigned int lane = threadIdx.x & 63;
    const double *ptr[NCH];
    unsigned int cnt[NCH], str[NCH], off[NCH];
    const double *safe = &c.st->zero;
#pragma unroll
    for (int i = 0; i < NCH; ++i)
        {
        const bool on = i < (int)c.n_cv && c.src[i].partials != nullptr;
        ptr[i] = on ? c.src[i].partials : safe;
        cnt[i] = on ? c.src[i].n_partials : 0u;
        str[i] = on ? c.src[i].stride : 0u;
        off[i] = on ? c.src[i].offset : 0u;
        }
    const int ok = c.st->patch_valid;
    int org[CHAIN_MAX_CV];
#pragma unroll
    for (int i = 0; i < CHAIN_MAX_CV; ++i) org[i] = c.st->patch_org[i];
#pragma unroll
    for (int i = 0; i < NCH; ++i)
#pragma unroll
        for (int j = 0; j < 4; ++j)
            {
            const unsigned int b = lane + j * MTD_WAVE;
            const double *q = (SUMS && b < cnt[i]) ? ptr[i] + ((size_t)b * str[i] + off[i]) : safe;
            p.x[i][j] = SUMS ? *q : 0.0;
            }
    p.patch_ok = ok;
#pragma unroll
    for (int i = 0; i < CHAIN_MAX_CV; ++i) p.patch.org[i] = org[i];
    p.patch.v[0] = c.st->patch_v[lane];
#pragma unroll
    for (int r = 1; r < 4; ++r) p.patch.v[r] = NCH == 3 ? c.st->patch_v[min(lane + 64 * r, 215u)] : 0.0;
    }

__device__ __forceinline__ double chain_div(const MetadCfg &c, const double a, const double b, const double y)
    {
    if (!c.fastdiv) return a / b;
    const double q0 = a * y;
    const double r0 = __builtin_fma(-b, q0, a);
    const double q1 = __builtin_fma(r0, y, q0);
    const double r1 = __builtin_fma(-b, q1, a);
    return __builtin_fma(r1, y, q1);
    }

__device__ __forceinline__ ChainResult chain_wave(const MetadCfg &c, const bool deposit, const bool closed_form,
                                                  const CommK *rx = nullptr, const double *given = nullptr,
                                                  const bool want_weight = false, const GridPatch *patch = nullptr,
                                                  const bool patch_ok = true, const bool have_init = false,
                                                  const double v_init0 = 0.0, const double v_init1 = 0.0, const double v_init2 = 0.0)
    {
    const int lane = threadIdx.x & 63;
    const unsigned int n = c.n_cv;
    const int n_term = 1 << n;
    ChainResult r;

    double x[CHAIN_MAX_CV][8];
    unsigned int n_part_max = 0;
#pragma unroll
    for (int i = 0; i < CHAIN_MAX_CV; ++i)
        if (i < (int)n && c.src[i].partials) n_part_max = max(n_part_max, c.src[i].n_partials);
    double v[CHAIN_MAX_CV] = { 0.0, 0.0, 0.0 };
    double rx_total[3] = { 0.0, 0.0, 0.0 };
    if (rx)
        {
        comm_recv_sum_wave(*rx, rx_total, n);
        n_part_max = 0;
        }
    else if (given)
        {
#pragma unroll
        for (int i = 0; i < CHAIN_MAX_CV; ++i) rx_total[i] = i < (int)n ? given[i] : 0.0;
        n_part_max = 0;
        }
    const bool handed = rx != nullptr || given != nullptr;
    if (have_init && n_part_max)
        {
        v[0] = v_init0;
        v[1] = v_init1;
        v[2] = v_init2;
        }
    for (unsigned int b0 = lane + ((have_init && n_part_max) ? 4 * MTD_WAVE : 0); b0 < n_part_max; b0 += 8 * MTD_WAVE)
        {
#pragma unroll
        for (int i = 0; i < CHAIN_MAX_CV; ++i)
#pragma unroll
            for (int j = 0; j < 8; ++j)
                {
                const unsigned int b = b0 + j * MTD_WAVE;
                x[i][j] = (i < (int)n && c.src[i].partials && b < c.src[i].n_partials)
                              ? c.src[i].partials[(size_t)b * c.src[i].stride + c.src[i].offset] : 0.0;
                }
#pragma unroll
        for (int i = 0; i < CHAIN_MAX_CV; ++i)
            v[i] += ((x[i][0] + x[i][1]) + (x[i][2] + x[i][3])) + ((x[i][4] + x[i][5]) + (x[i][6] + x[i][7]));
        }
#pragma unroll
    for (int i = 0; i < CHAIN_MAX_CV; ++i)
        {
        r.cv[i] = 0.0;
        r.bias[i] = 0.0;
        if (i < (int)n)
            {
            const double t = handed ? rx_total[i] : wave_sum(v[i]);
            r.cv[i] = (c.src[i].partials || handed) ? c.src[i].shift + c.src[i].scale * t : c.src[i].shift;
            }
        }

    MTD_STAMP(40, blockIdx.x == 0 && threadIdx.x == 0 && closed_form);
    int g_lower = 0, g_ok = 0;
    double g_rel = 0.0;
    if (lane < 3 * (int)n)
        {
        const int i = lane / 3, v = lane % 3;
        const double si = i == 0 ? r.cv[0] : (i == 1 ? r.cv[1] : r.cv[2]);
        const double delta = i == 0 ? c.delta[0] : (i == 1 ? c.delta[1] : c.delta[2]);
        const double cmin = i == 0 ? c.cv_min[0] : (i == 1 ? c.cv_min[1] : c.cv_min[2]);
        const double cmax = i == 0 ? c.cv_max[0] : (i == 1 ? c.cv_max[1] : c.cv_max[2]);
        const double rdel = i == 0 ? c.rdelta[0] : (i == 1 ? c.rdelta[1] : c.rdelta[2]);
        const int len = (int)(i == 0 ? c.lengths[0] : (i == 1 ? c.lengths[1] : c.lengths[2]));
        double val = si;
        if (v == 0) val = si - delta;
        if (v == 2) val = si + delta;
        g_ok = val >= cmin && val < cmax;
        int lower = (int)chain_div(c, val - cmin, delta, rdel);
        int upper = lower + 1;
        if (upper >= len)
            {
            lower--;
            upper--;
            }
        const double lower_bound = cmin + delta * lower;
        const double upper_bound = cmin + delta * upper;
        g_rel = (val - lower_bound) / (upper_bound - lower_bound);
        g_lower = lower;
        }

    MTD_STAMP(41, blockIdx.x == 0 && threadIdx.x == 0 && closed_form);
    const int n_pts = closed_form ? 1 + 2 * (int)n : 2 + 2 * (int)n;
    const int p = lane / n_term;
    const unsigned int bits = lane % n_term;
    const bool is_weight = (!closed_form) && p == 1 + 2 * (int)n;
    bool ok = p < n_pts;
    double wt = 1.0;
    unsigned int cell = 0;
    double d[CHAIN_MAX_CV];
    int pslot = 0, pmul = 1;
    bool in_patch = patch != nullptr && patch_ok;
#pragma unroll
    for (int i = 0; i < CHAIN_MAX_CV; ++i)
        {
        d[i] = 0.0;
        if (i < (int)n)
            {
            int var = 1;
            if (p == 1 + 2 * i) var = 0;
            if (p == 2 + 2 * i) var = 2;
            const int src_lane = 3 * i + var;
            const int lower = __shfl(g_lower, src_lane, MTD_WAVE);
            const double rel = __shfl(g_rel, src_lane, MTD_WAVE);
            const int oki = __shfl(g_ok, src_lane, MTD_WAVE);
            ok = ok && oki;
            unsigned int coord;
            if (bits & (1u << i))
                {
                coord = (unsigned int)lower;
                wt *= (1.0 - rel);
                }
            else
                {
                coord = (unsigned int)(lower + 1);
                wt *= rel;
                }
            cell += coord * c.factors[i];
            d[i] = (c.cv_min[i] + coord * c.delta[i]) - r.cv[i];
            if (patch)
                {
                const int o = (int)coord - patch->org[i];
                in_patch = in_patch && o >= 0 && o < 6;
                pslot += o * pmul;
                pmul *= 6;
                }
            }
        }
    double val = 0.0;
    if (patch)
        {
        const int src = (in_patch && ok) ? pslot : 0;
        double pv = __shfl(patch->v[0], src & 63, MTD_WAVE);
        if (n == 3)
            {
            const double p1 = __shfl(patch->v[1], src & 63, MTD_WAVE), p2 = __shfl(patch->v[2], src & 63, MTD_WAVE),
                         p3 = __shfl(patch->v[3], src & 63, MTD_WAVE);
            const int reg = src >> 6;
            pv = reg == 0 ? pv : (reg == 1 ? p1 : (reg == 2 ? p2 : p3));
            }
        if (ok) val = (in_patch && !is_weight) ? pv : (is_weight ? c.weight[cell] : c.grid[cell]);
        }
    else if (ok) val = is_weight ? c.weight[cell] : c.grid[cell];
    r.c_wt = wt;
    r.c_wold = (want_weight && ok && p == 0) ? c.weight[cell] : 0.0;
    r.c_dV = 0.0;

    double e_g = 0.0;
    if (closed_form && deposit && ok)
        {
        double gauss_exp = 0.0;
#pragma unroll
        for (int i = 0; i < CHAIN_MAX_CV; ++i)
#pragma unroll
            for (int j = 0; j < CHAIN_MAX_CV; ++j)
                if (i < (int)n && j < (int)n)
                    {
                    const double sij = c.sigma_inv[i * n + j];
                    gauss_exp += d[i] * d[j] * (1.0 / 2.0) * (sij * sij);
                    }
        e_g = exp(-gauss_exp);
        }
    bool on_grid = true;
    unsigned int bin = 0;
#pragma unroll
    for (int i = 0; i < CHAIN_MAX_CV; ++i)
        {
        if (i < (int)n)
            {
            const double q = chain_div(c, r.cv[i] - c.cv_min[i], c.delta[i], c.rdelta[i]);
            if (!(q > -1.0) || !(q < 4294967296.0))
                on_grid = false;
            else
                {
                const unsigned int coord = (unsigned int)q;
                if (coord >= c.lengths[i]) on_grid = false;
                bin += coord * c.factors[i];
                }
            }
        }
    r.on_grid = on_grid ? 1 : 0;
    r.bin = bin;

    MTD_STAMP(42, blockIdx.x == 0 && threadIdx.x == 0 && closed_form);
    double term = ok ? wt * val : 0.0;
    double V_old = 0.0;
    for (int b = 0; b < n_term; ++b) V_old += wave_read(term, b);
    r.scal = 1.0;
    if (deposit && c.mode == MTD_MODE_WELL_TEMPERED) r.scal = exp(chain_div(c, -V_old, c.T_shift, c.rT_shift));

    MTD_STAMP(43, blockIdx.x == 0 && threadIdx.x == 0 && closed_form);
    if (closed_form && deposit && ok)
        {
        r.c_dV = (c.W * r.scal) * e_g;
        val += r.c_dV;
        term = wt * val;
        }
    if (!ok) r.c_wt = 0.0;

    MTD_STAMP(44, blockIdx.x == 0 && threadIdx.x == 0 && closed_form);
    double res = 0.0;
    if (n == 2)
        {
        res += dpp_move<0x00>(term);
        res += dpp_move<0x55>(term);
        res += dpp_move<0xAA>(term);
        res += dpp_move<0xFF>(term);
        }
    else if (n == 1)
        {
        res += dpp_move<0xA0>(term);
        res += dpp_move<0xF5>(term);
        }
    else
        {
        const int base = (p < n_pts ? p : 0) * n_term;
        double t8[8];
#pragma unroll
        for (int b = 0; b < 8; ++b) t8[b] = __shfl(term, (base + b) & 63, MTD_WAVE);
#pragma unroll
        for (int b = 0; b < 8; ++b) res += t8[b];
        }

    const double res0 = wave_read(res, 0);
    r.V = res0;
    r.w = closed_form ? 1.0 : wave_read(res, (1 + 2 * (int)n) * n_term);
    r.oob = !wave_read((int)ok, 0);
#pragma unroll
    for (int i = 0; i < CHAIN_MAX_CV; ++i)
        {
        if (i < (int)n)
            {
            const double rm = wave_read(res, (1 + 2 * i) * n_term);
            const double rp = wave_read(res, (2 + 2 * i) * n_term);
            const double s = r.cv[i];
            const double delta = c.delta[i];
            double b;
            if (s - delta < c.cv_min[i])
                b = chain_div(c, rp - res0, delta, c.rdelta[i]);
            else if (s + delta > c.cv_max[i])
                b = chain_div(c, res0 - rm, delta, c.rdelta[i]);
            else
                b = chain_div(c, rp - rm, 2.0 * delta, c.rdelta2[i]);
            r.bias[i] = b;
            }
        }
    MTD_STAMP(45, blockIdx.x == 0 && threadIdx.x == 0 && closed_form);
    r.failed = 0;
    if (handed)
        {
        bool bad = false;
#pragma unroll
        for (int i = 0; i < CHAIN_MAX_CV; ++i) bad = bad || (i < (int)n && is_comm_poison(rx_total[i]));
        if (bad)
            {
            const double nan = __longlong_as_double(0x7ff8000000000000ll);
#pragma unroll
            for (int i = 0; i < CHAIN_MAX_CV; ++i)
                if (i < (int)n) r.cv[i] = r.bias[i] = nan;
            r.V = r.w = nan;
            r.scal = 0.0;
            r.on_grid = 0;
            r.oob = 0;
            r.failed = 1;
            }
        }
    return r;
    }

__device__ __forceinline__ double gauss_exponent3(const MetadCfg &c, unsigned int idx, const double s0, const double s1,
                                                  const double s2)
    {
    const unsigned int n = c.n_cv;
    unsigned int rest = idx;
    unsigned int c2 = 0, c1 = 0, c0;
    if (n > 2)
        {
        c2 = rest / c.factors[2];
        rest -= c2 * c.factors[2];
        }
    if (n > 1)
        {
        c1 = rest / c.factors[1];
        rest -= c1 * c.factors[1];
        }
    c0 = rest;
    double d[3];
    d[0] = (c.cv_min[0] + c0 * c.delta[0]) - s0;
    d[1] = n > 1 ? (c.cv_min[1] + c1 * c.delta[1]) - s1 : 0.0;
    d[2] = n > 2 ? (c.cv_min[2] + c2 * c.delta[2]) - s2 : 0.0;
    double gauss_exp = 0.0;
#pragma unroll
    for (int i = 0; i < 3; ++i)
#pragma unroll
        for (int j = 0; j < 3; ++j)
            if (i < (int)n && j < (int)n)
                {
                const double sij = c.sigma_inv[i * n + j];
                gauss_exp += d[i] * d[j] * (1.0 / 2.0) * (sij * sij);
                }
    return gauss_exp;
    }


__device__ __forceinline__ void chain_share(ChainResult &s_chain, const ChainResult &r)
    {
    s_chain.cv[0] = r.cv[0]; s_chain.cv[1] = r.cv[1]; s_chain.cv[2] = r.cv[2];
    s_chain.bias[0] = r.bias[0]; s_chain.bias[1] = r.bias[1]; s_chain.bias[2] = r.bias[2];
    s_chain.scal = r.scal; s_chain.V = r.V; s_chain.w = r.w;
    s_chain.bin = r.bin; s_chain.on_grid = r.on_grid; s_chain.oob = r.oob; s_chain.failed = r.failed;
    }

__device__ __forceinline__ double2 grid_first_pass_cell(const MetadCfg &c, const ChainResult &s_chain, const unsigned int g)
    {
    const double dV = (c.W * s_chain.scal) * exp(-gauss_exponent3(c, g, s_chain.cv[0], s_chain.cv[1], s_chain.cv[2]));
    c.grid_delta[g] = dV;
    unsigned int hd = c.hist_delta[g];
    if (s_chain.on_grid && g == s_chain.bin)
        {
        hd += 1;
        c.hist_delta[g] = hd;
        c.sigma_grid_delta[g] += c.det_sigma;
        c.hist_gauss_delta[g] += 1;
        }
    const double Rw = c.rew[g] + (double)hd;
    c.rew[g] = Rw;
    return make_double2(Rw * dV, Rw);
    }

__device__ __forceinline__ double2 grid_first_pass_cells_256(const MetadCfg &c, const ChainResult &s_chain, const unsigned int vb)
    {
    const bool mine = threadIdx.x < 256;
    const unsigned int g = vb * 256 + threadIdx.x;
    double2 s = make_double2(0.0, 0.0);
    if (mine && g < c.len && !s_chain.failed) s = grid_first_pass_cell(c, s_chain, g);
    return s;
    }

__device__ __forceinline__ void grid_first_pass_sums_256(const MetadCfg &c, const unsigned int vb, const double2 s, double *s_red)
    {
    const unsigned int wave = threadIdx.x >> 6, lane = threadIdx.x & 63;
    const double s1 = wave_sum(s.x), s2 = wave_sum(s.y);
    if (threadIdx.x < 256 && lane == 0)
        {
        s_red[2 * wave] = s1;
        s_red[2 * wave + 1] = s2;
        }
    __syncthreads();
    if (threadIdx.x == 0)
        {
        double t1 = 0.0, t2 = 0.0;
        for (int w = 0; w < 4; ++w)
            {
            t1 += s_red[2 * w];
            t2 += s_red[2 * w + 1];
            }
        c.gpart[2 * vb] = t1;
        c.gpart[2 * vb + 1] = t2;
        }
    }

__device__ __forceinline__ void grid_first_pass_256(const MetadCfg &c, const ChainResult &s_chain, const unsigned int vb, double *s_red)
    {
    grid_first_pass_sums_256(c, vb, grid_first_pass_cells_256(c, s_chain, vb), s_red);
    }

__device__ __forceinline__ void publish_step(const MetadCfg &c, const ChainResult &s_chain, const int deposit, const double *given = nullptr,
                                             const CommK *rx = nullptr)
    {
    const int lane = threadIdx.x & 63;
    double w_now = 1.0;
    if (!deposit) w_now = chain_wave(c, false, false, rx, given).w;
    if (lane < (int)c.n_cv)
        {
        const double s_l = lane == 0 ? s_chain.cv[0] : (lane == 1 ? s_chain.cv[1] : s_chain.cv[2]);
        c.st->cv[lane] = s_l;
        c.st->bias[lane] = lane == 0 ? s_chain.bias[0] : (lane == 1 ? s_chain.bias[1] : s_chain.bias[2]);
        const double dl = lane == 0 ? c.delta[0] : (lane == 1 ? c.delta[1] : c.delta[2]);
        const double ml = lane == 0 ? c.cv_min[0] : (lane == 1 ? c.cv_min[1] : c.cv_min[2]);
        const double ll = (double)(lane == 0 ? c.lengths[0] : (lane == 1 ? c.lengths[1] : c.lengths[2]));
        double q = (s_l - ml) / dl;
        if (!(q > 0.0)) q = 0.0;
        if (q > ll) q = ll;
        c.st->guess_org[lane] = (int)q - 2;
        }
    if (lane == 0)
        {
        c.st->V = s_chain.V;
        c.st->failed = (unsigned int)s_chain.failed;
        c.st->bin = s_chain.bin;
        c.st->on_grid = (unsigned int)s_chain.on_grid;
        if (deposit)
            c.st->scal = s_chain.scal;
        else
            {
            c.st->w = s_chain.failed ? s_chain.V : w_now;
            if (s_chain.on_grid) c.hist_delta[s_chain.bin] += 1;
            }
        if (s_chain.oob) c.st->n_oob += (deposit && c.mode == MTD_MODE_WELL_TEMPERED) ? 2 : 1;
        }
    }

}
```

metadynamics-plugin_amd/csrc/steinhardt.hip:

```cpp
#include "mtd_device.hpp"
#include "steinhardt_device.hpp"
#include "metad_host.hpp"

#include <cmath>
#include <cstring>
#include <map>
#include <mutex>

namespace
{

using namespace mtd;

constexpr int QL_THREADS = 256;
constexpr unsigned int QL_MAX_BLOCKS = 1024;


constexpr int QL_PPB = 64, QL_CAP = 1024, QL_K = QL_CAP / QL_THREADS;
static_assert(QL_PPB == MTD_WAVE, "one wave scans the neighbour counts of a chunk");
static_assert(QL_K == 4 && QL_PPB <= 256, "owner bytes of a thread's entries packed in one register");

struct QlUnit
    {
    unsigned int start[QL_PPB];
// ... 381 lines not shown
#pragma unroll
            for (int i = 0; i < MTD_WAVE / 4; ++i) sum += red[v * QL_RED_STRIDE + quarter * (MTD_WAVE / 4) + i];
            }
        part[quarter * QL_RED + v] = sum;
        __builtin_amdgcn_fence(__ATOMIC_RELEASE, "wavefront");
        __builtin_amdgcn_wave_barrier();
        __builtin_amdgcn_fence(__ATOMIC_ACQUIRE, "wavefront");
        if (lane < QL_RED && r * QL_RED + (int)lane < 2 * NLM)
            s_row[r * QL_RED + lane] = (part[lane] + part[QL_RED + lane]) + (part[2 * QL_RED + lane] + part[3 * QL_RED + lane]);
        __builtin_amdgcn_fence(__ATOMIC_RELEASE, "wavefront");
        __builtin_amdgcn_wave_barrier();
        __builtin_amdgcn_fence(__ATOMIC_ACQUIRE, "wavefront");
        }
    }

template<int LMAX> constexpr int ql_acc_roles() { return LMAX <= 8 ? 1 : 2; }

#ifdef MTD_QL_ACC_OCC
template<int LMAX, bool EVEN> constexpr int ql_acc_blocks_per_cu() { return MTD_QL_ACC_OCC; }
#else
template<int LMAX, bool EVEN> constexpr int ql_acc_blocks_per_cu() { return LMAX <= 6 ? (EVEN ? 3 : 2) : (LMAX <= 8 && EVEN ? 2 : 1); }
#endif

template<typename S4, int LMAX, bool SYM, bool EVEN>
__global__ __launch_bounds__(QL_THREADS, (ql_acc_blocks_per_cu<LMAX, EVEN>())) void k_ql_accumulate(const QlArgs<LMAX> a, const S4 *__restrict__ postype,
                                                                 const unsigned int *__restrict__ head_list,
                                                                 const unsigned int *__restrict__ n_neigh,
                                                                 const unsigned int *__restrict__ nlist, double *__restrict__ partials,
                                                                 const double *__restrict__ tab)
    {
    constexpr int NLM = (LMAX + 1) * (LMAX + 2) / 2;
    constexpr int NROLES = ql_acc_roles<LMAX>();
    __shared__ double s_wave[QL_THREADS / MTD_WAVE][2 * NLM];
    __shared__ __attribute__((aligned(16))) unsigned char s_raw[QL_ACC_LDS];
    QlAccPipe &pipe = *reinterpret_cast<QlAccPipe *>(s_raw);
    const int wave = threadIdx.x >> 6;
    double *red = reinterpret_cast<double *>(s_raw) + (size_t)wave * (QL_RED * QL_RED_STRIDE + 64);
    if (NROLES == 1)
        ql_accumulate_role<S4, LMAX, 0, 1, SYM, EVEN>(a, postype, head_list, n_neigh, nlist, tab, pipe, red, s_wave[wave]);
    else if (wave & 1)
        ql_accumulate_role<S4, LMAX, 1, 2, SYM, EVEN>(a, postype, head_list, n_neigh, nlist, tab, pipe, red, s_wave[wave]);
    else
        ql_accumulate_role<S4, LMAX, 0, 2, SYM, EVEN>(a, postype, head_list, n_neigh, nlist, tab, pipe, red, s_wave[wave]);
    __syncthreads();
    const unsigned int n_out = (a.lmax + 1) * (a.lmax + 2);
    for (unsigned int q = threadIdx.x; q < n_out; q += blockDim.x)
        {
        double v = 0.0;
        for (int w = 0; w < QL_THREADS / MTD_WAVE; ++w) v += s_wave[w][q];
        partials[(size_t)blockIdx.x * n_out + q] = v * fabs(tab[QlTab<LMAX>::NRM + q / 2]);
        }
    }

template<int LMAX>
__global__ __launch_bounds__(256) void k_ql_finalize(const QlArgs<LMAX> a, const double *__restrict__ qprime,
                                                     double *__restrict__ qlm_full, double *__restrict__ ql, double *__restrict__ value);

template<int LMAX>
__global__ __launch_bounds__(256) void k_ql_finalize_carrier(const QlArgs<LMAX> a, const double *__restrict__ qprime,
                                                             double *__restrict__ qlm_full, double *__restrict__ ql,
                                                             double *__restrict__ value, const mtd::MetadCfg cfg);

template<int LMAX>
__device__ __forceinline__ void ql_finalize_body(const QlArgs<LMAX> &a, const double *__restrict__ qprime,
                                                 double *__restrict__ qlm_full, double *__restrict__ ql, double *__restrict__ value,
                                                 const bool write = true, double *s_value = nullptr)
    {
    __shared__ double s_sq[(LMAX + 1) * (LMAX + 1)];
    __shared__ double s_ql[LMAX + 1];
    const double ng = (double)a.n_global;
    const unsigned int n = threadIdx.x;
    const unsigned int count = (a.lmax + 1) * (a.lmax + 1);
    if (n < count)
        {
        int l = 0;
        while ((l + 1) * (l + 1) <= (int)n) ++l;
        const int p = (int)n - l * l;
        const int m = (p <= l) ? p : (l - p);
        const int am = m < 0 ? -m : m;
        const int idx = l * (l + 1) / 2 + am;
        cplx q = {qprime[2 * idx], qprime[2 * idx + 1]};
        if (m < 0) q = cconj(q);
        if (m > 0 && (m % 2)) q = cscale(q, -1.0);
        if (a.half_nlist)
            {
            if (l % 2 == 0)
                q = cscale(q, 2.0);
            else
                q = {0.0, 0.0};
            }
        if (write)
            {
            qlm_full[2 * n] = q.re;
            qlm_full[2 * n + 1] = q.im;
            }
        double sq = q.re * q.re + q.im * q.im;
        sq *= (4.0 * M_PI / (2 * l + 1)) / (ng * ng);
        s_sq[n] = sq;
        }
    __syncthreads();
    if (threadIdx.x <= a.lmax)
        {
        const int l = threadIdx.x;
        double Ql = 0.0;
        for (int p = 0; p < 2 * l + 1; ++p) Ql += s_sq[l * l + p];
        if (write) ql[l] = Ql;
        s_ql[l] = Ql;
        }
    __syncthreads();
    if (threadIdx.x == 0)
        {
        double val = 0.0;
        for (int l = 0; l <= (int)a.lmax; ++l) val += a.ql_ref[l] * s_ql[l];
        if (write) *value = val;
        if (s_value) *s_value = val;
        }
    }

template<int LMAX>
__global__ __launch_bounds__(256) void k_ql_finalize(const QlArgs<LMAX> a, const double *__restrict__ qprime,
                                                     double *__restrict__ qlm_full, double *__restrict__ ql, double *__restrict__ value)
    {
    ql_finalize_body<LMAX>(a, qprime, qlm_full, ql, value);
    }

template<int LMAX>
__global__ __launch_bounds__(256) void k_ql_finalize_carrier(const QlArgs<LMAX> a, const double *__restrict__ qprime,
                                                             double *__restrict__ qlm_full, double *__restrict__ ql,
                                                             double *__restrict__ value, const mtd::MetadCfg cfg)
    {
    if (blockIdx.x > 0)
        {
        __shared__ double s_red[16];
        const unsigned int c0 = (blockIdx.x - 1) * 256;
        mtd::apply_cells(cfg, c0, min(cfg.len, c0 + 256u), blockIdx.x == 1, s_red);
        return;
        }
    ql_finalize_body<LMAX>(a, qprime, qlm_full, ql, value);
    }

template<int LMAX>
__global__ __launch_bounds__(256) void k_ql_finalize_chain(const QlArgs<LMAX> a, const double *__restrict__ qprime,
                                                           double *__restrict__ qlm_full, double *__restrict__ ql,
                                                           double *__restrict__ value, const mtd::MetadCfg c, const int deposit,
                                                           const unsigned int n_grid_blocks)
    {
    using namespace mtd;
    __shared__ double s_given[3];
    __shared__ ChainResult s_chain;
    __shared__ double s_red[16];
    const int wave = threadIdx.x >> 6, lane = threadIdx.x & 63;
    ChainPre<1> pre;
    if (wave == 0) chain_preload<1, false>(c, pre);
    if (threadIdx.x < 3) s_given[threadIdx.x] = 0.0;
    ql_finalize_body<LMAX>(a, qprime, qlm_full, ql, value, blockIdx.x == 0, &s_given[0]);
    __syncthreads();
    if (wave == 0)
        {
        const ChainResult r = chain_wave(c, deposit != 0, true, nullptr, s_given, false, &pre.patch, pre.patch_ok != 0);
        if (lane == 0) chain_share(s_chain, r);
        }
    __syncthreads();
    if (blockIdx.x < n_grid_blocks) grid_first_pass_256(c, s_chain, blockIdx.x, s_red);
    if (blockIdx.x == 0 && wave == 0) publish_step(c, s_chain, deposit, s_given);
    }

constexpr int QL_BINS = 4;
constexpr int QL_BIN_BITS = 48;
constexpr int QL_BIN_LOW = -120;
constexpr size_t QL_ACC_WORDS = 3 * QL_BINS + 1;

__device__ __forceinline__ void ql_exact_add(unsigned long long *acc , const int comp, double x)
    {
    if (!(fabs(x) < 4722366482869645213696.0))
        {
        const unsigned int bit = x != x ? 4u : (x > 0.0 ? 1u : 2u);
        atomicOr((unsigned int *)(acc + 3 * QL_BINS), bit << (4 * comp));
        return;
        }
#pragma unroll
    for (int k = QL_BINS - 1; k >= 0; --k)
        {
        const int w = QL_BIN_LOW + QL_BIN_BITS * k;
        const double t = trunc(ldexp(x, -w));
        if (t != 0.0)
            {
            atomicAdd(acc + comp * QL_BINS + k, (unsigned long long)(long long)t);
            x -= ldexp(t, w);
            }
        }
    }

template<typename S4>
__global__ __launch_bounds__(256) void k_ql_exact_to_force(const unsigned long long *__restrict__ acc, const double *__restrict__ own, const unsigned int N,
                                                           S4 *__restrict__ force)
    {
    typedef typename scalar4_traits<S4>::scalar scalar;
    const unsigned int i = blockIdx.x * blockDim.x + threadIdx.x;
    if (i >= N) return;
    const unsigned long long *a = acc + (size_t)i * QL_ACC_WORDS;
    const unsigned int flags = (unsigned int)a[3 * QL_BINS];
    double f[3];
#pragma unroll
    for (int c = 0; c < 3; ++c)
        {
        double v = 0.0;
#pragma unroll
        for (int k = 0; k < QL_BINS; ++k) v += ldexp((double)(long long)a[c * QL_BINS + k], QL_BIN_LOW + QL_BIN_BITS * k);
        v += own[3 * (size_t)i + c];
        const unsigned int fl = (flags >> (4 * c)) & 7u;
        if (fl & 4u) v = nan("");
        if (fl & 1u) v += INFINITY;
        if (fl & 2u) v -= INFINITY;
        f[c] = v;
        }
    force[i] = scalar4_traits<S4>::make((scalar)f[0], (scalar)f[1], (scalar)f[2], (scalar)0);
    }


struct QlNoCarry { };
struct QlCarry { mtd::MetadCfg cfg; unsigned int n_apply; };
template<bool CARRY> struct QlCarryArg { typedef QlNoCarry type; };
template<> struct QlCarryArg<true> { typedef QlCarry type; };

template<typename S4, int LMAX, bool HALF, bool EXACT, bool CARRY = false>
__global__ __launch_bounds__(QL_THREADS, (LMAX <= 6 ? 3 : 2)) void k_ql_forces(const QlArgs<LMAX> a, const S4 *__restrict__ postype,
                                                             const unsigned int *__restrict__ head_list,
                                                             const unsigned int *__restrict__ n_neigh,
                                                             const unsigned int *__restrict__ nlist, const double *__restrict__ qlm_full,
                                                             S4 *__restrict__ force, const double *__restrict__ d_bias, const double bias_host,
                                                             unsigned long long *__restrict__ exact_acc, double *__restrict__ own,
                                                             const double *__restrict__ tab, const typename QlCarryArg<CARRY>::type carry)
    {
    unsigned int n_work = gridDim.x;
    if constexpr (CARRY)
        {
        n_work = gridDim.x - carry.n_apply;
        if (blockIdx.x >= n_work)
            {
            __shared__ double s_red_apply[16];
            const unsigned int c0 = (blockIdx.x - n_work) * 256;
            mtd::apply_cells(carry.cfg, c0, min(carry.cfg.len, c0 + 256u), blockIdx.x == n_work, s_red_apply);
            return;
            }
        }
    typedef typename scalar4_traits<S4>::scalar scalar;
    constexpr int NLM = (LMAX + 1) * (LMAX + 2) / 2;
    constexpr unsigned int PPB = QL_PPB, CAP = QL_CAP;
    constexpr int K = QL_K;
    static_assert(QL_THREADS == 4 * QL_PPB, "four summing threads per particle");
    __shared__ double s_qw[2 * NLM];
    __shared__ QlUnit su[3];
    __shared__ double s_fx[CAP], s_fy[CAP], s_fz[CAP];
    const unsigned int tid = threadIdx.x;
    const bool setup_wave = (tid >> 6) == QL_THREADS / MTD_WAVE - 1;
    const double bias = d_bias ? *d_bias : bias_host;
    const double ng = (double)a.n_global;
    unsigned int active_l = 0;
#pragma unroll
    for (int l = 0; l <= LMAX; ++l)
        if (l <= (int)a.lmax && a.ql_ref[l] != 0.0) active_l |= 1u << l;
    active_l = __builtin_amdgcn_readfirstlane(active_l);
    for (unsigned int q = tid; q < (unsigned int)NLM; q += blockDim.x)
        {
        int l = 0;
        while ((l + 1) * (l + 2) / 2 <= (int)q) ++l;
        const int m = (int)q - l * (l + 1) / 2;
        double re = 0.0, im = 0.0;
        if (l <= (int)a.lmax)
            {
            const double w = bias * (4.0 * M_PI / (2 * l + 1)) / (ng * ng) * a.ql_ref[l] * (m > 0 ? 4.0 : 2.0) * tab[QlTab<LMAX>::NRM + q];
            const int n = l * l + m;
            re = w * qlm_full[2 * n];
            im = -w * qlm_full[2 * n + 1];
            }
        s_qw[2 * q] = re;
        s_qw[2 * q + 1] = im;
        }
    QlFeed<S4, LMAX> feed(a, postype, head_list, n_neigh);
    feed.n_work = n_work;
    if (setup_wave) feed.template begin<2>(su);
    lds_barrier();
    unsigned int j_cur[K], j_next[K], own_cur, own_next;
    ql_request_entries(su[0], nlist, j_cur, own_cur);
    ql_request_entries(su[1], nlist, j_next, own_next);
    S4 pos_raw = zero_s4<S4>();
    if (su[0].valid && tid < min(su[0].total, CAP)) pos_raw = postype[j_cur[0]];
    double Fx = 0.0, Fy = 0.0, Fz = 0.0;

    for (unsigned int n = 0;; ++n)
        {
        const QlUnit &U = su[n % 3];
        if (!U.valid) break;
        const QlUnit &NU = su[(n + 1) % 3];
        const unsigned int base = U.base, total = U.total, chunk = U.chunk;
        const unsigned int n_cur = min(total - base, CAP);
        const unsigned int n_next = NU.valid ? min(NU.total - NU.base, CAP) : 0u;
        unsigned int j0 = j_cur[0], j1 = j_cur[1], j2 = j_cur[2], j3 = j_cur[3], owners = own_cur;
#pragma unroll 1
        for (int k = 0; k < K; ++k)
            {
            const unsigned int t = k * QL_THREADS + tid;
            unsigned int tab_shift = 0;
            asm volatile("" : "+s"(tab_shift));
            const double *__restrict__ tab_k = tab + tab_shift;
            const bool last = k == K - 1;
            const unsigned int jx = last ? j_next[0] : j1;
            const bool want = last ? tid < n_next : t + QL_THREADS < n_cur;
            S4 pos_ahead = zero_s4<S4>();
            if (want) pos_ahead = postype[jx];
            if (t < n_cur)
                {
                const unsigned int p = owners & 255u;
                const Particle pj = scalar4_traits<S4>::unpack(pos_raw);
                double dx = U.px[p] - pj.x, dy = U.py[p] - pj.y, dz = U.pz[p] - pj.z;
                min_image(a, dx, dy, dz);
                const double rsq = dx * dx + dy * dy + dz * dz;
// ... 712 lines not shown
```

Baseline: 110.3 billion particle-CV-evals/s.

## Specialise chain wave on grid dimension and pin config in scalar registers

Templates the bias chain evaluation (chain_wave, preload, publish_step) on the compile-time number of grid variables instead of the runtime n_cv, and preloads the metadynamics config into a ChainCfg struct whose fields are forced into scalar registers via readfirstlane. The fused force kernel also drops its second force-register set and evaluates the second particle group after storing the first, which lowers vector register pressure. The intent is to shorten the serial chain latency on wave 0 and relieve register pressure on the streaming waves. The cost is more kernel instantiations, and the second group's compute now starts only after the first group's store.

```diff
diff --git a/metadynamics-plugin_amd/csrc/fused.hip b/metadynamics-plugin_amd/csrc/fused.hip
--- a/metadynamics-plugin_amd/csrc/fused.hip
+++ b/metadynamics-plugin_amd/csrc/fused.hip
@@ -106,7 +106,7 @@
 template<> struct ff_groups<double4, 1, true> { static constexpr int value = 2; };
 template<> struct ff_groups<double4, 1, false> { static constexpr int value = 2; };
 
-template<typename S4, int NCV, bool FAST, int GROUPS, bool COMM, bool ORTHO>
+template<typename S4, int NCV, int NG, bool FAST, int GROUPS, bool COMM, bool ORTHO>
 __global__ __launch_bounds__(FF_THREADS, 4) void k_fused_force(const LamKArgs a, const S4 *__restrict__ postype, const ForcePtrs out,
                                                             const unsigned int N, const double two_over_n, const MetadCfg c,
                                                             const int deposit, const unsigned int n_grid_blocks, const CommK ck)
@@ -125,11 +125,11 @@
     const unsigned int first = block_id * FF_STREAM_THREADS + (wave - 1) * MTD_WAVE + lane;
     const unsigned int first1 = first + FF_U * stride;
 
-    ForceRegs<NCV, FF_U> R, R1;
+    ForceRegs<NCV, FF_U> R;
     MTD_STAMP(16, blockIdx.x == 0 && threadIdx.x == 0);
     MTD_STAMP(24, blockIdx.x == n_grid_blocks && threadIdx.x == 0);
-    constexpr int NCH = CHAIN_MAX_CV;
-    ChainPre<NCH> pre;
+    static_assert(NCV <= NG && NG <= CHAIN_MAX_CV, "the set's CVs are variables of the grid");
+    ChainPre<NG> pre;
     constexpr bool early = !COMM;
     float4 th = make_float4(0.f, 0.f, 0.f, 0.f), tq = th;
     float tc = 0.0f;
@@ -145,12 +145,14 @@
             if (lane < NCV * MTD_MAX_TYPES) tc = a.coeff[lane / MTD_MAX_TYPES][lane % MTD_MAX_TYPES];
             }
         if (early)
-            chain_preload<NCH>(c, pre);
+            chain_preload<NG>(c, pre);
         else
-            chain_preload<NCH, false>(c, pre);
-        }
-    RawGroup<S4, FF_U> raw0;
+            chain_preload<NG, false>(c, pre);
+        }
+    RawGroup<S4, FF_U> raw0, raw1;
     if (wave != 0 && !grid_block && N) lam_force_request<S4, FF_U>(postype, N, first, stride, raw0);
+    ChainCfg<NG> kc;
+    chain_cfg_load<NG>(c, kc);
     if (!grid_block)
         {
         if (wave == 0)
@@ -171,12 +173,11 @@
         if constexpr (early)
             {
             double vi[3];
-#pragma unroll
-            for (int i = 0; i < NCH; ++i) vi[i] = (pre.x[i][0] + pre.x[i][1]) + (pre.x[i][2] + pre.x[i][3]);
-            r = chain_wave(c, deposit != 0, true, nullptr, nullptr, false, &pre.patch, pre.patch_ok != 0, true, vi[0], vi[1], vi[2]);
+            chain_pre_sums<NG>(pre, vi);
+            r = chain_wave<NG>(c, kc, deposit != 0, true, nullptr, nullptr, false, &pre.patch, pre.patch_ok != 0, true, vi[0], vi[1], vi[2]);
             }
         else
-            r = chain_wave(c, deposit != 0, true, &ck, nullptr, false, &pre.patch, pre.patch_ok != 0);
+            r = chain_wave<NG>(c, kc, deposit != 0, true, &ck, nullptr, false, &pre.patch, pre.patch_ok != 0);
         MTD_STAMP(17, blockIdx.x == 0 && threadIdx.x == 0);
         MTD_STAMP(26, blockIdx.x == n_grid_blocks && threadIdx.x == 0);
         if (lane == 0) chain_share(s_chain, r);
@@ -190,10 +191,8 @@
         }
     else if (!grid_block && N)
         {
-        RawGroup<S4, FF_U> raw1;
         if (GROUPS > 1) lam_force_request<S4, FF_U>(postype, N, first1, stride, raw1);
         lam_force_unscaled_from<S4, NCV, FAST, FF_U, ORTHO>(a, N, first, stride, s_mt, raw0, R);
-        if (GROUPS > 1) lam_force_unscaled_from<S4, NCV, FAST, FF_U, ORTHO>(a, N, first1, stride, s_mt, raw1, R1);
         MTD_STAMP(27, blockIdx.x == n_grid_blocks && threadIdx.x == 64);
         }
     lds_barrier();
@@ -210,11 +209,17 @@
     else if (wave != 0 && N)
         {
         lam_force_store<S4, NCV, FF_U>(a, out, first, stride, s_wcoef, R);
-        if (GROUPS > 1) lam_force_store<S4, NCV, FF_U>(a, out, first1, stride, s_wcoef, R1);
+        if (GROUPS > 1)
+            {
+            MTD_STAMP(30, blockIdx.x == n_grid_blocks && threadIdx.x == 64);
+            lam_force_unscaled_from<S4, NCV, FAST, FF_U, ORTHO>(a, N, first1, stride, s_mt, raw1, R);
+            MTD_STAMP(31, blockIdx.x == n_grid_blocks && threadIdx.x == 64);
+            lam_force_store<S4, NCV, FF_U>(a, out, first1, stride, s_wcoef, R);
+            }
         MTD_STAMP(29, blockIdx.x == n_grid_blocks && threadIdx.x == 64);
         }
 
-    if (blockIdx.x == 0 && wave == 0) publish_step(c, s_chain, deposit, nullptr, COMM ? &ck : nullptr);
+    if (blockIdx.x == 0 && wave == 0) publish_step<NG>(c, s_chain, deposit, nullptr, COMM ? &ck : nullptr);
     }
 
 template<typename S4, bool FAST>
@@ -471,16 +476,21 @@
                 unsigned int fblocks = (n_particles + per_block - 1) / per_block;
                 if (fblocks == 0 && n_grid == 0) fblocks = 1;
                 const unsigned int grid = n_grid + fblocks;
-                dispatch_bool(m->comm != nullptr, [&](auto comm_c)
+                dispatch_count<CHAIN_MAX_CV>(m->cfg.n_cv, [&](auto n_grid_c)
                     {
-                    dispatch_bool(k.ortho != 0, [&](auto ortho_c)
+                    constexpr int NG = decltype(n_grid_c)::value < NCV ? NCV : decltype(n_grid_c)::value;
+                    dispatch_bool(m->comm != nullptr, [&](auto comm_c)
                         {
-                        const auto kernel = k_fused_force<S4, NCV, FAST, G, decltype(comm_c)::value, decltype(ortho_c)::value>;
-                        if (timed)
-                            hipExtLaunchKernelGGL(kernel, dim3(grid), dim3(FF_THREADS), 0, s, ev_start, ev_stop, 0, k, (const S4 *)d_postype, out,
-                                                  n_particles, two_over_n, m->cfg, dep, n_grid, ck);
-                        else
-                            kernel<<<grid, FF_THREADS, 0, s>>>(k, (const S4 *)d_postype, out, n_particles, two_over_n, m->cfg, dep, n_grid, ck);
+                        constexpr bool COMM = decltype(comm_c)::value && NG == NCV;
+                        dispatch_bool(k.ortho != 0, [&](auto ortho_c)
+                            {
+                            const auto kernel = k_fused_force<S4, NCV, NG, FAST, G, COMM, decltype(ortho_c)::value>;
+                            if (timed)
+                                hipExtLaunchKernelGGL(kernel, dim3(grid), dim3(FF_THREADS), 0, s, ev_start, ev_stop, 0, k, (const S4 *)d_postype, out,
+                                                      n_particles, two_over_n, m->cfg, dep, n_grid, ck);
+                            else
+                                kernel<<<grid, FF_THREADS, 0, s>>>(k, (const S4 *)d_postype, out, n_particles, two_over_n, m->cfg, dep, n_grid, ck);
+                            });
                         });
                     });
                 });
@@ -570,9 +580,9 @@
     std::memset(&ck, 0, sizeof(ck));
     switch (m->cfg.n_cv)
         {
-        case 1: k_fused_force<float4, 1, true, 1, false, false><<<grid, FF_THREADS, 0, s>>>(k, nullptr, out, 0, 0.0, m->cfg, dep, n_grid, ck); break;
-        case 2: k_fused_force<float4, 2, true, 1, false, false><<<grid, FF_THREADS, 0, s>>>(k, nullptr, out, 0, 0.0, m->cfg, dep, n_grid, ck); break;
-        default: k_fused_force<float4, 3, true, 1, false, false><<<grid, FF_THREADS, 0, s>>>(k, nullptr, out, 0, 0.0, m->cfg, dep, n_grid, ck); break;
+        case 1: k_fused_force<float4, 1, 1, true, 1, false, false><<<grid, FF_THREADS, 0, s>>>(k, nullptr, out, 0, 0.0, m->cfg, dep, n_grid, ck); break;
+        case 2: k_fused_force<float4, 2, 2, true, 1, false, false><<<grid, FF_THREADS, 0, s>>>(k, nullptr, out, 0, 0.0, m->cfg, dep, n_grid, ck); break;
+        default: k_fused_force<float4, 3, 3, true, 1, false, false><<<grid, FF_THREADS, 0, s>>>(k, nullptr, out, 0, 0.0, m->cfg, dep, n_grid, ck); break;
         }
     MTD_LAUNCH_CHECK();
     m->pending_apply = dep;
diff --git a/metadynamics-plugin_amd/csrc/fused_step.hip b/metadynamics-plugin_amd/csrc/fused_step.hip
--- a/metadynamics-plugin_amd/csrc/fused_step.hip
+++ b/metadynamics-plugin_amd/csrc/fused_step.hip
@@ -231,6 +231,8 @@
         X.ok = has_extra && ix < p1;
         if (N && has_extra) raw_x = postype[X.ok ? ix : N - 1];
         }
+    ChainCfg<NCV> kc;
+    chain_cfg_load<NCV>(c, kc);
     load_coeff(a, s_coeff);
     load_modes_cv(a, s_cvt);
     load_modes(a, s_mt, true);
@@ -313,7 +315,7 @@
         MTD_STAMP(4, blockIdx.x == 0 && threadIdx.x == 0); MTD_STAMP(20, blockIdx.x == gridDim.x - 1 && threadIdx.x == 0);
         if (lane == 0) MTD_BSTAMP(2);
         if (COMM && b == 0) comm_send_wave(ck, tot, NS);
-        const ChainResult r = chain_wave(c, deposit != 0, closed, COMM ? &ck : nullptr, COMM ? nullptr : tot, b == 0 && deposit != 0, &patch);
+        const ChainResult r = chain_wave<NCV>(c, kc, deposit != 0, closed, COMM ? &ck : nullptr, COMM ? nullptr : tot, b == 0 && deposit != 0, &patch);
         c_wt = r.c_wt; c_wold = r.c_wold; c_dV = r.c_dV;
         MTD_STAMP(5, blockIdx.x == 0 && threadIdx.x == 0); MTD_STAMP(21, blockIdx.x == gridDim.x - 1 && threadIdx.x == 0);
         if (lane == 0) MTD_BSTAMP(3);
diff --git a/metadynamics-plugin_amd/csrc/mesh.hip b/metadynamics-plugin_amd/csrc/mesh.hip
--- a/metadynamics-plugin_amd/csrc/mesh.hip
+++ b/metadynamics-plugin_amd/csrc/mesh.hip
@@ -1411,7 +1411,7 @@
 constexpr int TFC_STREAM_THREADS = TF_THREADS - MTD_WAVE;
 constexpr int TFC_U = 4;
 
-template<typename S4, int NCV, bool FAST>
+template<typename S4, int NCV, int NG, bool FAST>
 __global__ __launch_bounds__(TF_THREADS, 4) void k_tile_forces_chain(const MeshGeom g, const TileGeom tg, const TileLists L,
                                                                   const double *__restrict__ mode, const double4 *__restrict__ packed,
                                                                   const double *__restrict__ inv, S4 *__restrict__ force,
@@ -1434,8 +1434,7 @@
     __shared__ unsigned short s_gx[TP_X + 2];
     const int wave = threadIdx.x >> 6, lane = threadIdx.x & 63;
 
-    constexpr int NCH = CHAIN_MAX_CV;
-    ChainPre<NCH> pre;
+    ChainPre<NG> pre;
     float4 th = make_float4(0.f, 0.f, 0.f, 0.f), tq = th;
     float tc = 0.0f;
     if (wave == 0)
@@ -1446,8 +1445,10 @@
             tq = a.q[lane];
             }
         if (lane < NCV * MTD_MAX_TYPES) tc = a.coeff[lane / MTD_MAX_TYPES][lane % MTD_MAX_TYPES];
-        chain_preload<NCH>(c, pre);
-        }
+        chain_preload<NG>(c, pre);
+        }
+    ChainCfg<NG> kc;
+    chain_cfg_load<NG>(c, kc);
     const unsigned int sid = threadIdx.x - MTD_WAVE;
     const unsigned int stride = gridDim.x * TFC_STREAM_THREADS;
     const unsigned int first = blockIdx.x * TFC_STREAM_THREADS + sid;
@@ -1503,9 +1504,8 @@
     if (wave == 0)
         {
         double vi[3];
-#pragma unroll
-        for (int i = 0; i < NCH; ++i) vi[i] = (pre.x[i][0] + pre.x[i][1]) + (pre.x[i][2] + pre.x[i][3]);
-        const ChainResult r = chain_wave(c, deposit != 0, true, nullptr, nullptr, false, &pre.patch, pre.patch_ok != 0, true, vi[0], vi[1], vi[2]);
+        chain_pre_sums<NG>(pre, vi);
+        const ChainResult r = chain_wave<NG>(c, kc, deposit != 0, true, nullptr, nullptr, false, &pre.patch, pre.patch_ok != 0, true, vi[0], vi[1], vi[2]);
         if (lane == 0) chain_share(s_chain, r);
         if (lane < NCV * MTD_MAX_TYPES)
             {
@@ -1534,7 +1534,7 @@
             }
         }
     if (blockIdx.x < n_grid_blocks) grid_first_pass_256(c, s_chain, blockIdx.x, s_red);
-    if (blockIdx.x == 0 && wave == 0) publish_step(c, s_chain, deposit);
+    if (blockIdx.x == 0 && wave == 0) publish_step<NG>(c, s_chain, deposit);
     if (!work) return;
     const double bias = mesh_slot == 0 ? s_chain.bias[0] : (mesh_slot == 1 ? s_chain.bias[1] : s_chain.bias[2]);
     const double s = two_over_n * bias;
@@ -3982,11 +3982,13 @@
     const double two_over_n = 2.0 / (double)n_global;
     const bool fast = n_lam ? mtd::lam_fast_trig(k) != 0 : true;
     const unsigned int n_stream = n_lam ? n_particles : 0u;
-#define MTD_LAUNCH_TFC(S4, NCV, FASTV) \
-    k_tile_forces_chain<S4, NCV, FASTV><<<blocks, TF_THREADS, 0, s>>>(g, mesh->tg, mesh->lists, mesh->d_mode, mesh->d_packed, mesh->d_inv, (S4 *)d_force_mesh, \
+#define MTD_LAUNCH_TFC(S4, NCV, NG, FASTV) \
+    k_tile_forces_chain<S4, NCV, NG, FASTV><<<blocks, TF_THREADS, 0, s>>>(g, mesh->tg, mesh->lists, mesh->d_mode, mesh->d_packed, mesh->d_inv, (S4 *)d_force_mesh, \
         two_over_n, mesh->n_types, mesh_slot, k, (const S4 *)d_postype, out, n_stream, m->cfg, dep, n_grid)
 #define MTD_LAUNCH_TFC_NCV(S4, FASTV) \
-    switch (n_lam) { case 0: case 1: MTD_LAUNCH_TFC(S4, 1, FASTV); break; case 2: MTD_LAUNCH_TFC(S4, 2, FASTV); break; default: MTD_LAUNCH_TFC(S4, 3, FASTV); break; }
+    switch (n_lam < 2 ? m->cfg.n_cv : 4u)  \
+        { case 1: MTD_LAUNCH_TFC(S4, 1, 1, FASTV); break; case 2: MTD_LAUNCH_TFC(S4, 1, 2, FASTV); break; case 3: MTD_LAUNCH_TFC(S4, 1, 3, FASTV); break; \
+          default: MTD_LAUNCH_TFC(S4, 2, 3, FASTV); break; }
     if (dtype == MTD_F32)
         {
         if (fast) { MTD_LAUNCH_TFC_NCV(float4, true) } else { MTD_LAUNCH_TFC_NCV(float4, false) }
diff --git a/metadynamics-plugin_amd/csrc/metad_device.hpp b/metadynamics-plugin_amd/csrc/metad_device.hpp
--- a/metadynamics-plugin_amd/csrc/metad_device.hpp
+++ b/metadynamics-plugin_amd/csrc/metad_device.hpp
@@ -3,6 +3,8 @@
 #include "mtd_device.hpp"
 #include "comm_device.hpp"
 #include "exact_div.hpp"
+
+#include <utility>
 
 #ifndef MTD_STAMP
 #define MTD_STAMP(slot, cond) do { } while (0)
@@ -415,24 +417,88 @@
     return gp;
     }
 
-template<int NCH> struct ChainPre
-    {
-    double x[NCH][4];
+template<int N> struct ChainCfg
+    {
+    double cv_min[N], cv_max[N], delta[N], rdelta[N], rdelta2[N];
+    unsigned int lengths[N], factors[N];
+    double scale[N], shift[N];
+    unsigned int has_partials[N];
+    unsigned int n_partials[N];
+    double sigma_inv[N * N];
+    double W, T_shift, rT_shift;
+    int mode, fastdiv;
+    const double *grid, *weight;
+    };
+
+__device__ __forceinline__ void chain_pin(unsigned int &x)
+    {
+    x = (unsigned int)__builtin_amdgcn_readfirstlane((int)x);
+    asm volatile("" : "+s"(x));
+    }
+__device__ __forceinline__ void chain_pin(int &x)
+    {
+    x = __builtin_amdgcn_readfirstlane(x);
+    asm volatile("" : "+s"(x));
+    }
+__device__ __forceinline__ void chain_pin(double &x)
+    {
+    x = __hiloint2double(__builtin_amdgcn_readfirstlane(__double2hiint(x)), __builtin_amdgcn_readfirstlane(__double2loint(x)));
+    asm volatile("" : "+s"(x));
+    }
+__device__ __forceinline__ void chain_pin(const double *&x)
+    {
+    const unsigned long long p = (unsigned long long)x;
+    const unsigned int lo = (unsigned int)__builtin_amdgcn_readfirstlane((int)(unsigned int)p),
+                       hi = (unsigned int)__builtin_amdgcn_readfirstlane((int)(unsigned int)(p >> 32));
+    x = (const double *)(((unsigned long long)hi << 32) | lo);
+    asm volatile("" : "+s"(x));
+    }
+
+template<int N, int... I, int... IJ>
+__device__ __forceinline__ void chain_cfg_load_seq(const MetadCfg &c, ChainCfg<N> &k, std::integer_sequence<int, I...>,
+                                                   std::integer_sequence<int, IJ...>)
+    {
+    ((k.cv_min[I] = c.cv_min[I], k.cv_max[I] = c.cv_max[I], k.delta[I] = c.delta[I], k.rdelta[I] = c.rdelta[I],
+      k.rdelta2[I] = c.rdelta2[I], k.lengths[I] = c.lengths[I], k.factors[I] = c.factors[I], k.scale[I] = c.src[I].scale,
+      k.shift[I] = c.src[I].shift,
+      k.has_partials[I] = (unsigned int)(unsigned long long)c.src[I].partials | (unsigned int)((unsigned long long)c.src[I].partials >> 32),
+      k.n_partials[I] = c.src[I].n_partials), ...);
+    ((k.sigma_inv[IJ] = N < 3 ? c.sigma_inv[IJ] : 0.0), ...);
+    k.W = c.W; k.T_shift = c.T_shift; k.rT_shift = c.rT_shift;
+    k.mode = c.mode; k.fastdiv = c.fastdiv;
+    k.grid = c.grid; k.weight = c.weight;
+    ((chain_pin(k.cv_min[I]), chain_pin(k.cv_max[I]), chain_pin(k.delta[I]), chain_pin(k.rdelta[I]), chain_pin(k.rdelta2[I]),
+      chain_pin(k.lengths[I]), chain_pin(k.factors[I]), chain_pin(k.scale[I]), chain_pin(k.shift[I]), chain_pin(k.has_partials[I]),
+      chain_pin(k.n_partials[I])), ...);
+    if constexpr (N < 3) (chain_pin(k.sigma_inv[IJ]), ...);
+    chain_pin(k.W); chain_pin(k.T_shift); chain_pin(k.rT_shift); chain_pin(k.mode); chain_pin(k.fastdiv);
+    chain_pin(k.grid); chain_pin(k.weight);
+    }
+
+template<int N> __device__ __forceinline__ void chain_cfg_load(const MetadCfg &c, ChainCfg<N> &k)
+    {
+    static_assert(N >= 1 && N <= 3, "the chain handles one to three variables");
+    chain_cfg_load_seq<N>(c, k, std::make_integer_sequence<int, N>{}, std::make_integer_sequence<int, N * N>{});
+    }
+
+template<int N> struct ChainPre
+    {
+    double x[N][4];
     GridPatch patch;
     int patch_ok;
     };
 
-template<int NCH, bool SUMS = true>
-__device__ __forceinline__ void chain_preload(const MetadCfg &c, ChainPre<NCH> &p)
+template<int N, bool SUMS = true>
+__device__ __forceinline__ void chain_preload(const MetadCfg &c, ChainPre<N> &p)
     {
     const unsigned int lane = threadIdx.x & 63;
-    const double *ptr[NCH];
-    unsigned int cnt[NCH], str[NCH], off[NCH];
+    const double *ptr[N];
+    unsigned int cnt[N], str[N], off[N];
     const double *safe = &c.st->zero;
 #pragma unroll
-    for (int i = 0; i < NCH; ++i)
-        {
-        const bool on = i < (int)c.n_cv && c.src[i].partials != nullptr;
+    for (int i = 0; i < N; ++i)
+        {
+        const bool on = c.src[i].partials != nullptr;
         ptr[i] = on ? c.src[i].partials : safe;
         cnt[i] = on ? c.src[i].n_partials : 0u;
         str[i] = on ? c.src[i].stride : 0u;
@@ -443,7 +509,7 @@
 #pragma unroll
     for (int i = 0; i < CHAIN_MAX_CV; ++i) org[i] = c.st->patch_org[i];
 #pragma unroll
-    for (int i = 0; i < NCH; ++i)
+    for (int i = 0; i < N; ++i)
 #pragma unroll
         for (int j = 0; j < 4; ++j)
             {
@@ -456,12 +522,20 @@
     for (int i = 0; i < CHAIN_MAX_CV; ++i) p.patch.org[i] = org[i];
     p.patch.v[0] = c.st->patch_v[lane];
 #pragma unroll
-    for (int r = 1; r < 4; ++r) p.patch.v[r] = NCH == 3 ? c.st->patch_v[min(lane + 64 * r, 215u)] : 0.0;
-    }
-
-__device__ __forceinline__ double chain_div(const MetadCfg &c, const double a, const double b, const double y)
-    {
-    if (!c.fastdiv) return a / b;
+    for (int r = 1; r < 4; ++r) p.patch.v[r] = N == 3 ? c.st->patch_v[min(lane + 64 * r, 215u)] : 0.0;
+    }
+
+template<int N> __device__ __forceinline__ void chain_pre_sums(const ChainPre<N> &p, double *vi)
+    {
+#pragma unroll
+    for (int i = 0; i < CHAIN_MAX_CV; ++i) vi[i] = 0.0;
+#pragma unroll
+    for (int i = 0; i < N; ++i) vi[i] = (p.x[i][0] + p.x[i][1]) + (p.x[i][2] + p.x[i][3]);
+    }
+
+__device__ __forceinline__ double chain_div(const bool fast, const double a, const double b, const double y)
+    {
+    if (!fast) return a / b;
     const double q0 = a * y;
     const double r0 = __builtin_fma(-b, q0, a);
     const double q1 = __builtin_fma(r0, y, q0);
@@ -469,33 +543,48 @@
     return __builtin_fma(r1, y, q1);
     }
 
-__device__ __forceinline__ ChainResult chain_wave(const MetadCfg &c, const bool deposit, const bool closed_form,
+template<int N> __device__ __forceinline__ double chain_sigma_inv(const MetadCfg &c, const ChainCfg<N> &k, const int ij)
+    {
+    if constexpr (N < 3)
+        return k.sigma_inv[ij];
+    else
+        return c.sigma_inv[ij];
+    }
+
+template<typename T, int N> __device__ __forceinline__ T chain_sel(const T (&a)[N], const int i)
+    {
+    const T a0 = a[0], a1 = a[N > 1 ? 1 : 0], a2 = a[N > 2 ? 2 : 0];
+    return i == 0 ? a0 : (i == 1 ? a1 : a2);
+    }
+
+template<int N>
+__device__ __forceinline__ ChainResult chain_wave(const MetadCfg &c, const ChainCfg<N> &k, const bool deposit, const bool closed_form,
                                                   const CommK *rx = nullptr, const double *given = nullptr,
                                                   const bool want_weight = false, const GridPatch *patch = nullptr,
                                                   const bool patch_ok = true, const bool have_init = false,
                                                   const double v_init0 = 0.0, const double v_init1 = 0.0, const double v_init2 = 0.0)
     {
     const int lane = threadIdx.x & 63;
-    const unsigned int n = c.n_cv;
-    const int n_term = 1 << n;
+    constexpr int n_term = 1 << N;
+    const bool fast = k.fastdiv != 0;
     ChainResult r;
 
-    double x[CHAIN_MAX_CV][8];
+    double x[N][8];
     unsigned int n_part_max = 0;
 #pragma unroll
-    for (int i = 0; i < CHAIN_MAX_CV; ++i)
-        if (i < (int)n && c.src[i].partials) n_part_max = max(n_part_max, c.src[i].n_partials);
+    for (int i = 0; i < N; ++i)
+        if (k.has_partials[i]) n_part_max = max(n_part_max, k.n_partials[i]);
     double v[CHAIN_MAX_CV] = { 0.0, 0.0, 0.0 };
     double rx_total[3] = { 0.0, 0.0, 0.0 };
     if (rx)
         {
-        comm_recv_sum_wave(*rx, rx_total, n);
+        comm_recv_sum_wave(*rx, rx_total, (unsigned int)N);
         n_part_max = 0;
         }
     else if (given)
         {
 #pragma unroll
-        for (int i = 0; i < CHAIN_MAX_CV; ++i) rx_total[i] = i < (int)n ? given[i] : 0.0;
+        for (int i = 0; i < N; ++i) rx_total[i] = given[i];
         n_part_max = 0;
         }
     const bool handed = rx != nullptr || given != nullptr;
@@ -508,16 +597,16 @@
     for (unsigned int b0 = lane + ((have_init && n_part_max) ? 4 * MTD_WAVE : 0); b0 < n_part_max; b0 += 8 * MTD_WAVE)
         {
 #pragma unroll
-        for (int i = 0; i < CHAIN_MAX_CV; ++i)
+        for (int i = 0; i < N; ++i)
 #pragma unroll
             for (int j = 0; j < 8; ++j)
                 {
                 const unsigned int b = b0 + j * MTD_WAVE;
-                x[i][j] = (i < (int)n && c.src[i].partials && b < c.src[i].n_partials)
+                x[i][j] = (c.src[i].partials && b < c.src[i].n_partials)
                               ? c.src[i].partials[(size_t)b * c.src[i].stride + c.src[i].offset] : 0.0;
                 }
 #pragma unroll
-        for (int i = 0; i < CHAIN_MAX_CV; ++i)
+        for (int i = 0; i < N; ++i)
             v[i] += ((x[i][0] + x[i][1]) + (x[i][2] + x[i][3])) + ((x[i][4] + x[i][5]) + (x[i][6] + x[i][7]));
         }
 #pragma unroll
@@ -525,30 +614,31 @@
         {
         r.cv[i] = 0.0;
         r.bias[i] = 0.0;
-        if (i < (int)n)
-            {
-            const double t = handed ? rx_total[i] : wave_sum(v[i]);
-            r.cv[i] = (c.src[i].partials || handed) ? c.src[i].shift + c.src[i].scale * t : c.src[i].shift;
-            }
+        }
+#pragma unroll
+    for (int i = 0; i < N; ++i)
+        {
+        const double t = handed ? rx_total[i] : wave_sum(v[i]);
+        r.cv[i] = (k.has_partials[i] || handed) ? k.shift[i] + k.scale[i] * t : k.shift[i];
         }
 
     MTD_STAMP(40, blockIdx.x == 0 && threadIdx.x == 0 && closed_form);
     int g_lower = 0, g_ok = 0;
     double g_rel = 0.0;
-    if (lane < 3 * (int)n)
+    if (lane < 3 * N)
         {
         const int i = lane / 3, v = lane % 3;
         const double si = i == 0 ? r.cv[0] : (i == 1 ? r.cv[1] : r.cv[2]);
-        const double delta = i == 0 ? c.delta[0] : (i == 1 ? c.delta[1] : c.delta[2]);
-        const double cmin = i == 0 ? c.cv_min[0] : (i == 1 ? c.cv_min[1] : c.cv_min[2]);
-        const double cmax = i == 0 ? c.cv_max[0] : (i == 1 ? c.cv_max[1] : c.cv_max[2]);
-        const double rdel = i == 0 ? c.rdelta[0] : (i == 1 ? c.rdelta[1] : c.rdelta[2]);
-        const int len = (int)(i == 0 ? c.lengths[0] : (i == 1 ? c.lengths[1] : c.lengths[2]));
+        const double delta = chain_sel(k.delta, i);
+        const double cmin = chain_sel(k.cv_min, i);
+        const double cmax = chain_sel(k.cv_max, i);
+        const double rdel = chain_sel(k.rdelta, i);
+        const int len = (int)chain_sel(k.lengths, i);
         double val = si;
         if (v == 0) val = si - delta;
         if (v == 2) val = si + delta;
         g_ok = val >= cmin && val < cmax;
-        int lower = (int)chain_div(c, val - cmin, delta, rdel);
+        int lower = (int)chain_div(fast, val - cmin, delta, rdel);
         int upper = lower + 1;
         if (upper >= len)
             {
@@ -562,50 +652,46 @@
         }
 
     MTD_STAMP(41, blockIdx.x == 0 && threadIdx.x == 0 && closed_form);
-    const int n_pts = closed_form ? 1 + 2 * (int)n : 2 + 2 * (int)n;
+    const int n_pts = closed_form ? 1 + 2 * N : 2 + 2 * N;
     const int p = lane / n_term;
     const unsigned int bits = lane % n_term;
-    const bool is_weight = (!closed_form) && p == 1 + 2 * (int)n;
+    const bool is_weight = (!closed_form) && p == 1 + 2 * N;
     bool ok = p < n_pts;
     double wt = 1.0;
     unsigned int cell = 0;
-    double d[CHAIN_MAX_CV];
+    double d[N];
     int pslot = 0, pmul = 1;
     bool in_patch = patch != nullptr && patch_ok;
 #pragma unroll
-    for (int i = 0; i < CHAIN_MAX_CV; ++i)
-        {
-        d[i] = 0.0;
-        if (i < (int)n)
-            {
-            int var = 1;
-            if (p == 1 + 2 * i) var = 0;
-            if (p == 2 + 2 * i) var = 2;
-            const int src_lane = 3 * i + var;
-            const int lower = __shfl(g_lower, src_lane, MTD_WAVE);
-            const double rel = __shfl(g_rel, src_lane, MTD_WAVE);
-            const int oki = __shfl(g_ok, src_lane, MTD_WAVE);
-            ok = ok && oki;
-            unsigned int coord;
-            if (bits & (1u << i))
-                {
-                coord = (unsigned int)lower;
-                wt *= (1.0 - rel);
-                }
-            else
-                {
-                coord = (unsigned int)(lower + 1);
-                wt *= rel;
-                }
-            cell += coord * c.factors[i];
-            d[i] = (c.cv_min[i] + coord * c.delta[i]) - r.cv[i];
-            if (patch)
-                {
-                const int o = (int)coord - patch->org[i];
-                in_patch = in_patch && o >= 0 && o < 6;
-                pslot += o * pmul;
-                pmul *= 6;
-                }
+    for (int i = 0; i < N; ++i)
+        {
+        int var = 1;
+        if (p == 1 + 2 * i) var = 0;
+        if (p == 2 + 2 * i) var = 2;
+        const int src_lane = 3 * i + var;
+        const int lower = __shfl(g_lower, src_lane, MTD_WAVE);
+        const double rel = __shfl(g_rel, src_lane, MTD_WAVE);
+        const int oki = __shfl(g_ok, src_lane, MTD_WAVE);
+        ok = ok && oki;
+        unsigned int coord;
+        if (bits & (1u << i))
+            {
+            coord = (unsigned int)lower;
+            wt *= (1.0 - rel);
+            }
+        else
+            {
+            coord = (unsigned int)(lower + 1);
+            wt *= rel;
+            }
+        cell += coord * k.factors[i];
+        d[i] = (k.cv_min[i] + coord * k.delta[i]) - r.cv[i];
+        if (patch)
+            {
+            const int o = (int)coord - patch->org[i];
+            in_patch = in_patch && o >= 0 && o < 6;
+            pslot += o * pmul;
+            pmul *= 6;
             }
         }
     double val = 0.0;
@@ -613,18 +699,18 @@
         {
         const int src = (in_patch && ok) ? pslot : 0;
         double pv = __shfl(patch->v[0], src & 63, MTD_WAVE);
-        if (n == 3)
+        if constexpr (N == 3)
             {
             const double p1 = __shfl(patch->v[1], src & 63, MTD_WAVE), p2 = __shfl(patch->v[2], src & 63, MTD_WAVE),
                          p3 = __shfl(patch->v[3], src & 63, MTD_WAVE);
             const int reg = src >> 6;
             pv = reg == 0 ? pv : (reg == 1 ? p1 : (reg == 2 ? p2 : p3));
             }
-        if (ok) val = (in_patch && !is_weight) ? pv : (is_weight ? c.weight[cell] : c.grid[cell]);
-        }
-    else if (ok) val = is_weight ? c.weight[cell] : c.grid[cell];
+        if (ok) val = (in_patch && !is_weight) ? pv : (is_weight ? k.weight[cell] : k.grid[cell]);
+        }
+    else if (ok) val = is_weight ? k.weight[cell] : k.grid[cell];
     r.c_wt = wt;
-    r.c_wold = (want_weight && ok && p == 0) ? c.weight[cell] : 0.0;
+    r.c_wold = (want_weight && ok && p == 0) ? k.weight[cell] : 0.0;
     r.c_dV = 0.0;
 
     double e_g = 0.0;
@@ -632,32 +718,28 @@
         {
         double gauss_exp = 0.0;
 #pragma unroll
-        for (int i = 0; i < CHAIN_MAX_CV; ++i)
-#pragma unroll
-            for (int j = 0; j < CHAIN_MAX_CV; ++j)
-                if (i < (int)n && j < (int)n)
-                    {
-                    const double sij = c.sigma_inv[i * n + j];
-                    gauss_exp += d[i] * d[j] * (1.0 / 2.0) * (sij * sij);
-                    }
+        for (int i = 0; i < N; ++i)
+#pragma unroll
+            for (int j = 0; j < N; ++j)
+                {
+                const double sij = chain_sigma_inv<N>(c, k, i * N + j);
+                gauss_exp += d[i] * d[j] * (1.0 / 2.0) * (sij * sij);
+                }
         e_g = exp(-gauss_exp);
         }
     bool on_grid = true;
     unsigned int bin = 0;
 #pragma unroll
-    for (int i = 0; i < CHAIN_MAX_CV; ++i)
-        {
-        if (i < (int)n)
-            {
-            const double q = chain_div(c, r.cv[i] - c.cv_min[i], c.delta[i], c.rdelta[i]);
-            if (!(q > -1.0) || !(q < 4294967296.0))
-                on_grid = false;
-            else
-                {
-                const unsigned int coord = (unsigned int)q;
-                if (coord >= c.lengths[i]) on_grid = false;
-                bin += coord * c.factors[i];
-                }
+    for (int i = 0; i < N; ++i)
+        {
+        const double q = chain_div(fast, r.cv[i] - k.cv_min[i], k.delta[i], k.rdelta[i]);
+        if (!(q > -1.0) || !(q < 4294967296.0))
+            on_grid = false;
+        else
+            {
+            const unsigned int coord = (unsigned int)q;
+            if (coord >= k.lengths[i]) on_grid = false;
+            bin += coord * k.factors[i];
             }
         }
     r.on_grid = on_grid ? 1 : 0;
@@ -666,14 +748,15 @@
     MTD_STAMP(42, blockIdx.x == 0 && threadIdx.x == 0 && closed_form);
     double term = ok ? wt * val : 0.0;
     double V_old = 0.0;
+#pragma unroll
     for (int b = 0; b < n_term; ++b) V_old += wave_read(term, b);
     r.scal = 1.0;
-    if (deposit && c.mode == MTD_MODE_WELL_TEMPERED) r.scal = exp(chain_div(c, -V_old, c.T_shift, c.rT_shift));
+    if (deposit && k.mode == MTD_MODE_WELL_TEMPERED) r.scal = exp(chain_div(fast, -V_old, k.T_shift, k.rT_shift));
 
     MTD_STAMP(43, blockIdx.x == 0 && threadIdx.x == 0 && closed_form);
     if (closed_form && deposit && ok)
         {
-        r.c_dV = (c.W * r.scal) * e_g;
+        r.c_dV = (k.W * r.scal) * e_g;
         val += r.c_dV;
         term = wt * val;
         }
@@ -681,14 +764,14 @@
 
     MTD_STAMP(44, blockIdx.x == 0 && threadIdx.x == 0 && closed_form);
     double res = 0.0;
-    if (n == 2)
+    if constexpr (N == 2)
         {
         res += dpp_move<0x00>(term);
         res += dpp_move<0x55>(term);
         res += dpp_move<0xAA>(term);
         res += dpp_move<0xFF>(term);
         }
-    else if (n == 1)
+    else if constexpr (N == 1)
         {
         res += dpp_move<0xA0>(term);
         res += dpp_move<0xF5>(term);
@@ -705,26 +788,23 @@
 
     const double res0 = wave_read(res, 0);
     r.V = res0;
-    r.w = closed_form ? 1.0 : wave_read(res, (1 + 2 * (int)n) * n_term);
+    r.w = closed_form ? 1.0 : wave_read(res, (1 + 2 * N) * n_term);
     r.oob = !wave_read((int)ok, 0);
 #pragma unroll
-    for (int i = 0; i < CHAIN_MAX_CV; ++i)
-        {
-        if (i < (int)n)
-            {
-            const double rm = wave_read(res, (1 + 2 * i) * n_term);
-            const double rp = wave_read(res, (2 + 2 * i) * n_term);
-            const double s = r.cv[i];
-            const double delta = c.delta[i];
-            double b;
-            if (s - delta < c.cv_min[i])
-                b = chain_div(c, rp - res0, delta, c.rdelta[i]);
-            else if (s + delta > c.cv_max[i])
-                b = chain_div(c, res0 - rm, delta, c.rdelta[i]);
-            else
-                b = chain_div(c, rp - rm, 2.0 * delta, c.rdelta2[i]);
-            r.bias[i] = b;
-            }
+    for (int i = 0; i < N; ++i)
+        {
+        const double rm = wave_read(res, (1 + 2 * i) * n_term);
+        const double rp = wave_read(res, (2 + 2 * i) * n_term);
+        const double s = r.cv[i];
+        const double delta = k.delta[i];
+        double b;
+        if (s - delta < k.cv_min[i])
+            b = chain_div(fast, rp - res0, delta, k.rdelta[i]);
+        else if (s + delta > k.cv_max[i])
+            b = chain_div(fast, res0 - rm, delta, k.rdelta[i]);
+        else
+            b = chain_div(fast, rp - rm, 2.0 * delta, k.rdelta2[i]);
+        r.bias[i] = b;
         }
     MTD_STAMP(45, blockIdx.x == 0 && threadIdx.x == 0 && closed_form);
     r.failed = 0;
@@ -732,13 +812,12 @@
         {
         bool bad = false;
 #pragma unroll
-        for (int i = 0; i < CHAIN_MAX_CV; ++i) bad = bad || (i < (int)n && is_comm_poison(rx_total[i]));
+        for (int i = 0; i < N; ++i) bad = bad || is_comm_poison(rx_total[i]);
         if (bad)
             {
             const double nan = __longlong_as_double(0x7ff8000000000000ll);
 #pragma unroll
-            for (int i = 0; i < CHAIN_MAX_CV; ++i)
-                if (i < (int)n) r.cv[i] = r.bias[i] = nan;
+            for (int i = 0; i < N; ++i) r.cv[i] = r.bias[i] = nan;
             r.V = r.w = nan;
             r.scal = 0.0;
             r.on_grid = 0;
@@ -846,13 +925,19 @@
     grid_first_pass_sums_256(c, vb, grid_first_pass_cells_256(c, s_chain, vb), s_red);
     }
 
+template<int N>
 __device__ __forceinline__ void publish_step(const MetadCfg &c, const ChainResult &s_chain, const int deposit, const double *given = nullptr,
                                              const CommK *rx = nullptr)
     {
     const int lane = threadIdx.x & 63;
     double w_now = 1.0;
-    if (!deposit) w_now = chain_wave(c, false, false, rx, given).w;
-    if (lane < (int)c.n_cv)
+    if (!deposit)
+        {
+        ChainCfg<N> k;
+        chain_cfg_load<N>(c, k);
+        w_now = chain_wave<N>(c, k, false, false, rx, given).w;
+        }
+    if (lane < N)
         {
         const double s_l = lane == 0 ? s_chain.cv[0] : (lane == 1 ? s_chain.cv[1] : s_chain.cv[2]);
         c.st->cv[lane] = s_l;
diff --git a/metadynamics-plugin_amd/csrc/steinhardt.hip b/metadynamics-plugin_amd/csrc/steinhardt.hip
--- a/metadynamics-plugin_amd/csrc/steinhardt.hip
+++ b/metadynamics-plugin_amd/csrc/steinhardt.hip
@@ -557,17 +557,19 @@
     const int wave = threadIdx.x >> 6, lane = threadIdx.x & 63;
     ChainPre<1> pre;
     if (wave == 0) chain_preload<1, false>(c, pre);
+    ChainCfg<1> kc;
+    chain_cfg_load<1>(c, kc);
     if (threadIdx.x < 3) s_given[threadIdx.x] = 0.0;
     ql_finalize_body<LMAX>(a, qprime, qlm_full, ql, value, blockIdx.x == 0, &s_given[0]);
     __syncthreads();
     if (wave == 0)
         {
-        const ChainResult r = chain_wave(c, deposit != 0, true, nullptr, s_given, false, &pre.patch, pre.patch_ok != 0);
+        const ChainResult r = chain_wave<1>(c, kc, deposit != 0, true, nullptr, s_given, false, &pre.patch, pre.patch_ok != 0);
         if (lane == 0) chain_share(s_chain, r);
         }
     __syncthreads();
     if (blockIdx.x < n_grid_blocks) grid_first_pass_256(c, s_chain, blockIdx.x, s_red);
-    if (blockIdx.x == 0 && wave == 0) publish_step(c, s_chain, deposit, s_given);
+    if (blockIdx.x == 0 && wave == 0) publish_step<1>(c, s_chain, deposit, s_given);
     }
 
 constexpr int QL_BINS = 4;
```

After: 107.4 billion particle-CV-evals/s. 0.973x the previous value.
